# DanielLin94144/E2E-ASR-Pytorch

Measured on AMD Instinct MI355X. Metric: audio frames/sec (fwd+bwd) LibriSpeech-100 joint CTC-att, higher is better.
Workload: dtype bf16; 1 GPU; config/librispeech_asr.yaml (vgg 0, 4xBiLSTM-320, joint CTC-att 0.5), B=16 x T=1200 x D=160 per GPU, L=180, delta+SpecAugment on GPU, fwd+losses+bwd+grad-allreduce+clip+Adadelta, dropout on; global_batch=16, frames_per_utt=1200, parallelism=dp1

## Files before the change

### e2e-asr-pytorch_amd/csrc/ctc.hip

```cpp
#include "common.h"

namespace {

struct CtcP {
    const float* lp;
    const int64_t* tgt;
    const int64_t* in_len;
    const int64_t* tgt_len;
    float* nll;
    float* loss;
    float* grad;
    float* alpha;
    float* beta;
    int B, T, V, L, Smax;
    float gscale;
};

__device__ __forceinline__ float lse2(float a, float b) {
    const float m = fmaxf(a, b);
    if (m == -INFINITY) return -INFINITY;
    return m + __logf(1.f + __expf(-fabsf(a - b)));
}

__device__ __forceinline__ float lse3(float a, float b, float c) {
    const float m = fmaxf(fmaxf(a, b), c);
    if (m == -INFINITY) return -INFINITY;
    const float md = __builtin_amdgcn_fmed3f(a, b, c), mn = fminf(fminf(a, b), c);
    return m + __logf(1.f + __expf(md - m) + __expf(mn - m));
}

constexpr int CTC_FCH = 8;
constexpr size_t CTC_GRAD_LDS = 60 * 1024;

__global__ __launch_bounds__(1024) void ctc_sweep_kernel(CtcP p, int CF) {
    extern __shared__ __attribute__((aligned(16))) unsigned char smem[];
    const int b = blockIdx.x, back = blockIdx.y;
    const int tid = threadIdx.x, NTH = blockDim.x;
    const int V = p.V, T = p.T;
    int tl = (int)p.tgt_len[b];
    tl = max(0, min(tl, p.L));
    const int S = 2 * tl + 1;
    int Tin = (int)p.in_len[b];
    Tin = max(0, min(Tin, T));
    int* ext = reinterpret_cast<int*>(smem);
    float* buf0 = reinterpret_cast<float*>(ext + p.Smax + 2) + 2;
    float* buf1 = buf0 + p.Smax + 6;
    float* s_lp = buf1 + p.Smax + 4;
    const float* lp = p.lp + (long)b * T * V;
    float* lat = (back ? p.beta : p.alpha) + (long)b * T * p.Smax;

    for (int s = tid; s < p.Smax + 2; s += NTH) ext[s] = (s < S && (s & 1)) ? (int)p.tgt[(long)b * p.L + (s >> 1)] : 0;
    for (int s = tid - 2; s < p.Smax + 2; s += NTH) { buf0[s] = -INFINITY; buf1[s] = -INFINITY; }
    __syncthreads();
    if (Tin == 0) {
        if (!back && tid == 0) {
            const float n = (tl == 0) ? 0.f : INFINITY;
            p.nll[b] = n;
        }
        return;
    }
    const int nwb = (p.L + 1 + 63) >> 6;
    const bool label = (tid >> 6) >= nwb;
    const int s = label ? 2 * (tid - 64 * nwb) + 1 : 2 * tid;
    const bool sok = s < S;
    const int sr = sok ? s : 0;
    const int e = sok ? ext[s] : 0;
    bool skip = false;
    if (sok && !back) skip = (s >= 2) && e != 0 && e != ext[s - 2];
    if (sok && back) skip = (s + 2 < S) && ext[s + 2] != 0 && ext[s + 2] != e;
    float* prev = buf0;
    float* cur = buf1;
    for (int c0 = 0; c0 < Tin; c0 += CF) {
        const int nf = min(CF, Tin - c0);
        const int tlo = back ? Tin - c0 - nf : c0;
        __syncthreads();
        for (int i = tid; i < nf * V; i += NTH) s_lp[i] = lp[(long)tlo * V + i];
        __syncthreads();
        for (int i = 0; i < nf; ++i) {
            const int t = back ? Tin - 1 - (c0 + i) : c0 + i;
            const float lpe = s_lp[(t - tlo) * V + e];
            float a;
            if (c0 + i == 0) {
                if (!back) a = (s == 0 || s == 1) ? lpe : -INFINITY;
                else       a = (s == S - 1 || s == S - 2) ? lpe : -INFINITY;
            } else {
                const int d1 = back ? 1 : -1;
                if (label) a = lse3(prev[sr], prev[sr + d1], skip ? prev[sr + 2 * d1] : -INFINITY);
                else       a = lse2(prev[sr], prev[sr + d1]);
                a += lpe;
            }
            if (sok) { cur[s] = a; lat[(long)t * p.Smax + s] = a; }
            __syncthreads();
            float* tmp = prev; prev = cur; cur = tmp;
        }
    }
    if (!back && tid == 0) {
        float ll = prev[S - 1];
        if (S > 1) ll = lse2(ll, prev[S - 2]);
        p.nll[b] = -ll;
    }
}

template <int FCH>
__global__ __launch_bounds__(1024) void ctc_grad_kernel(CtcP p) {
    extern __shared__ __attribute__((aligned(16))) unsigned char smem[];
    const int b = blockIdx.y, t0 = blockIdx.x * FCH;
    const int tid = threadIdx.x, NTH = blockDim.x, lane = tid & 63, wave = tid >> 6, nwave = NTH >> 6;
    const int V = p.V, T = p.T;
    int tl = (int)p.tgt_len[b];
    tl = max(0, min(tl, p.L));
    const int S = 2 * tl + 1;
    int Tin = (int)p.in_len[b];
    Tin = max(0, min(Tin, T));
    float* acc = reinterpret_cast<float*>(smem);
    float* blk = acc + FCH * V;
    const float* lp = p.lp + (long)b * T * V;
    float* grad = p.grad + (long)b * T * V;
    for (int i = tid; i < FCH * V; i += NTH) acc[i] = 0.f;
    const int s = tid;
    const bool sok = s < S;
    const int e = (sok && (s & 1)) ? (int)p.tgt[(long)b * p.L + (s >> 1)] : 0;
    const float nll = p.nll[b];
    const float scale = p.gscale / (float)(max(tl, 1) * p.B);
    if (blockIdx.x == 0 && blockIdx.y == 0 && tid == 0) {
        float sum = 0.f;
        for (int bb = 0; bb < p.B; ++bb) {
            int l = (int)p.tgt_len[bb];
            l = max(1, min(l, p.L));
            sum += p.nll[bb] / (float)(l * p.B);
        }
        *p.loss = sum;
    }
    float occ[FCH];
#pragma unroll
    for (int f = 0; f < FCH; ++f) {
        const int t = t0 + f;
        occ[f] = 0.f;
        if (sok && t < Tin) {
            const long li = ((long)b * T + t) * p.Smax + s;
            occ[f] = expf(p.alpha[li] + p.beta[li] - lp[(long)t * V + e] + nll);
        }
    }
    __syncthreads();
#pragma unroll
    for (int f = 0; f < FCH; ++f) {
        if (sok && (s & 1) && t0 + f < Tin) atomicAdd(&acc[f * V + e], occ[f]);
        const float bsum = wave_sum((sok && !(s & 1)) ? occ[f] : 0.f);
        if (lane == 0) blk[f * nwave + wave] = bsum;
    }
    __syncthreads();
    for (int i = tid; i < FCH * V; i += NTH) {
        const int f = i / V, v = i - f * V, t = t0 + f;
        if (t >= T) continue;
        float g = 0.f;
        if (t < Tin) {
            float a = acc[i];
            if (v == 0) for (int w = 0; w < nwave; ++w) a += blk[f * nwave + w];
            if (!(nll < INFINITY)) a = NAN;
            g = scale * (expf(lp[(long)t * V + v]) - a);
        }
        grad[(long)t * V + v] = g;
    }
}

}

extern "C" size_t asr_ctc_loss_workspace_bytes(int B, int T, int L) {
    return 2 * (size_t)B * T * (2 * (size_t)L + 1) * sizeof(float);
}

extern "C" int asr_ctc_loss(const float* logp, const int64_t* targets, const int64_t* input_len, const int64_t* target_len,
                            float* nll, float* loss, float* grad, int B, int T, int V, int L, float gscale,
                            void* workspace, size_t workspace_bytes, asr_stream_t stream) {
    ASR_REQUIRE(logp && targets && input_len && target_len && nll && loss && grad && workspace, ASR_E_ARG, "asr_ctc_loss: null pointer");
    ASR_REQUIRE(B > 0 && T > 0 && V > 1 && L > 0, ASR_E_ARG, "asr_ctc_loss: bad dims");
    ASR_REQUIRE(workspace_bytes >= asr_ctc_loss_workspace_bytes(B, T, L), ASR_E_ARG, "asr_ctc_loss: workspace too small");
    const int Smax = 2 * L + 1;
    float* wsf = (float*)workspace;
    CtcP p{logp, targets, input_len, target_len, nll, loss, grad, wsf, wsf + (size_t)B * T * Smax, B, T, V, L, Smax, gscale};
    ASR_REQUIRE(Smax <= 1024, ASR_E_UNSUPPORTED, "asr_ctc_loss: 2L+1=%d states exceed one workgroup", Smax);
    const int nthr = 64 * ((L + 1 + 63) / 64 + (L + 63) / 64);
    const size_t fixed = (size_t)(Smax + 2) * 4 + 2 * (size_t)(Smax + 6) * 4 + 16;
    int CF = (int)((60 * 1024 - fixed) / ((size_t)V * 4));
    ASR_REQUIRE(CF >= 1, ASR_E_UNSUPPORTED, "asr_ctc_loss: V=%d classes exceed the LDS budget: at most V=%d with 2L+1=%d states "
                "(one frame of log-probs beside the lattice buffers in 60 KB)", V, (int)((60 * 1024 - fixed) / 4), Smax);
    if (CF > T) CF = T;
    const size_t lds_s = fixed + (size_t)CF * V * 4;
    const size_t lds_g1 = (size_t)(V + nthr / 64) * 4;
    ASR_REQUIRE(lds_g1 <= CTC_GRAD_LDS, ASR_E_UNSUPPORTED, "asr_ctc_loss: V=%d classes exceed the %zu bytes of LDS of the gradient kernel",
                V, CTC_GRAD_LDS);
    int fch = CTC_FCH;
    while ((size_t)fch * lds_g1 > CTC_GRAD_LDS) fch >>= 1;
    hipStream_t st = (hipStream_t)stream;
    hipLaunchKernelGGL(ctc_sweep_kernel, dim3(B, 2), dim3(nthr), lds_s, st, p, CF);
    const dim3 gg(cdiv(T, fch), B);
    switch (fch) {
        case 8: hipLaunchKernelGGL(ctc_grad_kernel<8>, gg, dim3(nthr), 8 * lds_g1, st, p); break;
        case 4: hipLaunchKernelGGL(ctc_grad_kernel<4>, gg, dim3(nthr), 4 * lds_g1, st, p); break;
        case 2: hipLaunchKernelGGL(ctc_grad_kernel<2>, gg, dim3(nthr), 2 * lds_g1, st, p); break;
        default: hipLaunchKernelGGL(ctc_grad_kernel<1>, gg, dim3(nthr), lds_g1, st, p); break;
    }
    ASR_LAUNCH_CHECK("asr_ctc_loss");
    return ASR_OK;
}
```

### e2e-asr-pytorch_amd/csrc/decoder.hip

```cpp
#include "common.h"
#include "gemm_plan.h"
#include "decoder_internal.h"
#include <stdlib.h>
#include <initializer_list>
#include <type_traits>

namespace {

template <typename F> void with_bool(bool v, F&& f) { if (v) f(std::true_type{}); else f(std::false_type{}); }
template <typename F> void with_knmax_h16(int Kn, bool h16, F&& f) {
    with_bool(h16, [&](auto h) {
        if (Kn <= 4) f(std::integral_constant<int, 4>{}, h);
        else if (Kn <= 10) f(std::integral_constant<int, 10>{}, h);
        else f(std::integral_constant<int, 16>{}, h);
    });
}

__host__ __device__ inline int conv_parts(int nout) { const int p = 512 / nout; return p < 1 ? 1 : (p > 8 ? 8 : p); }

__device__ __forceinline__ float tanh_fast(float x) { return 1.f - 2.f * __builtin_amdgcn_rcpf(1.f + __expf(2.f * x)); }

template <int U> struct Stage {
    float v[U];
    template <typename L> __device__ __forceinline__ void load(int n, int tid, int nthr, L ld) {
// ... 1046 lines not shown
    o.ntp_max = pi.tiles_max;
    o.slots = take((size_t)d.B * (o.nte > o.ntp_max ? o.nte : o.ntp_max) * o.slot);
    o.pwork_bytes = pi.work_bytes;
    o.pwork = take(o.pwork_bytes / sizeof(float) + 64);
    o.dxin = take((size_t)d.B * d.L * XW);
    o.dkeypre = take((size_t)d.B * d.Tp * d.A);
    o.datt_next = take((size_t)d.B * d.Tp);
    o.dcf = take((size_t)d.NL * d.B * d.Dd);
    o.wq_t = take((size_t)d.Q * d.A);
    o.wslots = take((size_t)d.B * o.nch * d.Kn * taps);
    for (int l = 0; l < d.NL; ++l) o.wcat[l] = take((size_t)((l == 0 ? XW : d.Dd) + d.Dd) * 4 * d.Dd);
    o.total = off;
    return o;
}

int check_dims(const asr_dec_dims_t& d, const char* who) {
    ASR_REQUIRE(d.B > 0 && d.Tp > 0 && d.E > 0 && d.A > 0 && d.Dd > 0 && d.V > 1 && d.L > 0, ASR_E_ARG, "%s: bad dims", who);
    ASR_REQUIRE(d.NL >= 1 && d.NL <= ASR_MAX_DEC_LAYERS, ASR_E_UNSUPPORTED, "%s: %d decoder layers (max %d)", who, d.NL, ASR_MAX_DEC_LAYERS);
    ASR_REQUIRE(d.Q == d.Dd * d.NL, ASR_E_ARG, "%s: Q must equal Dd*NL", who);
    ASR_REQUIRE(d.Kn >= 1 && d.Kn <= 16, ASR_E_UNSUPPORTED, "%s: loc_kernel_num %d not in [1,16]", who, d.Kn);
    ASR_REQUIRE(d.Ks >= 0 && d.Ks <= 512, ASR_E_UNSUPPORTED, "%s: loc_kernel_size %d too large", who, d.Ks);
    ASR_REQUIRE(d.temperature > 0.f, ASR_E_ARG, "%s: temperature must be > 0", who);
    ASR_REQUIRE(d.Tp <= 12000, ASR_E_UNSUPPORTED, "%s: T'=%d exceeds the LDS row budget", who, d.Tp);
    return ASR_OK;
}

struct EnergyPlan { int tpw; dim3 grid; size_t lds; };
EnergyPlan energy_plan(const asr_dec_dims_t& d) {
    const int cand_small[] = {2, 4, 5, 8}, cand_big[] = {2, 4, 5};
    const int* cand = (d.Kn <= 4) ? cand_small : cand_big;
    const int nc = (d.Kn <= 4) ? 4 : (d.Kn <= 10 ? 3 : 2);
    int tpw = cand[nc - 1];
    for (int i = 0; i < nc; ++i)
        if ((long)d.B * cdiv(d.Tp, 8 * cand[i]) <= 256) { tpw = cand[i]; break; }
    EnergyPlan pl;
    pl.tpw = tpw;
    const int TE = 8 * tpw;
    pl.grid = dim3(cdiv(d.Tp, TE), d.B);
    int n[5];
    energy_regions(TE, d.Kn, d.Ks, d.A, n);
    n[4] = conv_parts(d.Kn * (TE / 4)) * d.Kn * TE;
    pl.lds = lds_bytes(n, 5);
    return pl;
}
void launch_energy(const DecP& p, int t, const EnergyPlan& pl, hipStream_t st) {
    with_knmax_h16(p.d.Kn, p.s.key16 != nullptr, [&](auto kn, auto h) {
        constexpr int KNMAX = decltype(kn)::value;
        constexpr bool H16 = decltype(h)::value;
        switch (pl.tpw) {
            case 2: hipLaunchKernelGGL((att_energy_kernel<KNMAX, 2, H16>), pl.grid, dim3(512), pl.lds, st, p, t); break;
            case 4: hipLaunchKernelGGL((att_energy_kernel<KNMAX, 4, H16>), pl.grid, dim3(512), pl.lds, st, p, t); break;
            case 5: if constexpr (KNMAX <= 10) { hipLaunchKernelGGL((att_energy_kernel<KNMAX, 5, H16>), pl.grid, dim3(512), pl.lds, st, p, t); } break;
            default: if constexpr (KNMAX <= 4) { hipLaunchKernelGGL((att_energy_kernel<KNMAX, 8, H16>), pl.grid, dim3(512), pl.lds, st, p, t); } break;
        }
    });
}

void launch_step(const DecP& p, int t, bool bf, const EnergyPlan& epl, bool embed, hipStream_t st) {
    const asr_dec_dims_t& d = p.d;
    if (embed)
        hipLaunchKernelGGL(embed_kernel, dim3(cdiv((long)d.B * d.Dd, 256)), dim3(256), 0, st, p.w.emb, p.s.tokens, p.s.xin, d.B, d.L, d.Dd,
                           d.Dd + d.E, t, 1, d.V);
    with_bool(bf, [&](auto b) { hipLaunchKernelGGL(dec_query_kernel<decltype(b)::value>, dim3(cdiv(d.A, 16)), dim3(256), 0, st, p, t); });
    launch_energy(p, t, epl, st);
    if (p.s.enc16 && (d.E & 3) == 0) hipLaunchKernelGGL(att_softmax_ctx_kernel<true>, dim3(cdiv(d.E, 64), d.B), dim3(256), sizeof(float) * d.Tp, st, p, t);
    else hipLaunchKernelGGL(att_softmax_ctx_kernel<false>, dim3(cdiv(d.E, 64), d.B), dim3(256), sizeof(float) * d.Tp, st, p, t);
    for (int l = 0; l < d.NL; ++l)
        with_bool(bf, [&](auto b) { hipLaunchKernelGGL(dec_cell_fwd_kernel<decltype(b)::value>, dim3(cdiv(d.Dd, 4)), dim3(256), 0, st, p, t, l); });
}

GemmCall key_call(const asr_dec_dims_t& d, const asr_dec_weights_t& w, const float* enc, float* key, int prec) {
    GemmCall c{enc, w.Wk, key, w.bk, d.B * d.Tp, d.A, d.E, d.E, d.E, d.A};
    c.act = ASR_ACT_TANH; c.prec = prec;
    return c;
}

}

extern "C" size_t asr_att_decoder_fwd_work_bytes(const asr_dec_dims_t* dims) {
    return dims ? dec_fwd_plan_info(*dims).work_bytes : 0;
}
extern "C" int asr_att_decoder_fwd_plan(const asr_dec_dims_t* dims) { return dims ? dec_fwd_plan_info(*dims).kind : 0; }
extern "C" int asr_att_decoder_bwd_plan(const asr_dec_dims_t* dims) { return dims ? dec_bwd_plan_info(*dims).kind : 0; }
extern "C" int asr_att_decoder_energy_plan(const asr_dec_dims_t* dims, int* knmax, int* tpw) {
    ASR_REQUIRE(dims && knmax && tpw, ASR_E_ARG, "asr_att_decoder_energy_plan: null pointer");
    const int rc = check_dims(*dims, "asr_att_decoder_energy_plan");
    if (rc != ASR_OK) return rc;
    with_knmax_h16(dims->Kn, false, [&](auto kn, auto) { *knmax = decltype(kn)::value; });
    *tpw = energy_plan(*dims).tpw;
    return ASR_OK;
}

static __global__ void dec_fwd_begin_kernel(unsigned* status, int has_block) {
    status[threadIdx.x] = 0u;
    if (has_block && threadIdx.x == 0) status[DEC_FWD_LAUNCHED_WORD] = 0u;
}

extern "C" int asr_att_decoder_fwd(const asr_dec_dims_t* dims, const asr_dec_weights_t* weights,
                                   const float* enc, const int64_t* enc_len, const int64_t* teacher, int teacher_ld,
                                   const asr_dec_state_t* state, int prec, asr_stream_t stream) {
    ASR_REQUIRE(dims && weights && enc && enc_len && state, ASR_E_ARG, "asr_att_decoder_fwd: null pointer");
    const asr_dec_dims_t& d = *dims;
    int rc = check_dims(d, "asr_att_decoder_fwd");
    if (rc != ASR_OK) return rc;
    hipStream_t st = (hipStream_t)stream;
    DecP p{d, *weights, *state, enc, enc_len};
    const bool bf = (prec == ASR_BF16);
    if (state->work && state->work_bytes >= 256)
        hipLaunchKernelGGL(dec_fwd_begin_kernel, dim3(1), dim3(64), 0, st, (unsigned*)state->work, state->work_bytes >= DEC_STATUS_BYTES ? 1 : 0);

    rc = gemm_run(key_call(d, *weights, enc, state->key, prec), st);
    if (rc != ASR_OK) return rc;
    if (state->key16) hipLaunchKernelGGL(cast_bf16_kernel, dim3(1024), dim3(256), 0, st, state->key, (unsigned short*)state->key16, (long)d.B * d.Tp * d.A);
    if (state->enc16) hipLaunchKernelGGL(cast_bf16_kernel, dim3(1024), dim3(256), 0, st, enc, (unsigned short*)state->enc16, (long)d.B * d.Tp * d.E);

    if (teacher) {
        hipLaunchKernelGGL(shift_tokens_kernel, dim3(cdiv(d.B * d.L, 256)), dim3(256), 0, st, teacher, state->tokens, d.B, d.L, teacher_ld);
        hipLaunchKernelGGL(embed_kernel, dim3(cdiv((long)d.B * d.L * d.Dd, 256)), dim3(256), 0, st, weights->emb, state->tokens,
                           state->xin, d.B, d.L, d.Dd, d.Dd + d.E, 0, d.L, d.V);
    } else {
        hipMemsetAsync(state->tokens, 0, sizeof(int64_t) * d.B * d.L, st);
    }

    const EnergyPlan epl = energy_plan(d);
    ASR_REQUIRE(epl.lds <= 64 * 1024, ASR_E_UNSUPPORTED, "asr_att_decoder_fwd: energy tile needs %zu B of LDS", epl.lds);
    int t_begin = 0;
    if (teacher && bf && state->work) {
        rc = dec_fwd_persistent(d, *weights, *state, enc, enc_len, state->work, state->work_bytes, st);
        if (rc < 0) return rc;
        if (rc == ASR_OK) t_begin = d.L;
    }
    for (int t = t_begin; t < d.L; ++t) {
        launch_step(p, t, bf, epl, !teacher, st);
        if (!teacher) hipLaunchKernelGGL(dec_greedy_kernel, dim3(d.B), dim3(256), 0, st, p, t);
    }
    ASR_LAUNCH_CHECK("asr_att_decoder_fwd");
    if (teacher) {
        GemmCall logits{state->hs + (size_t)(d.NL - 1) * d.Dd, weights->Wc, state->logits, weights->bc, d.B * d.L, d.V, d.Dd,
                        (long)d.NL * d.Dd, d.Dd, d.V};
        logits.prec = prec;
        rc = gemm_run(logits, st);
        if (rc != ASR_OK) return rc;
    }
    return ASR_OK;
}

extern "C" int asr_att_decoder_keys(const asr_dec_dims_t* dims, const asr_dec_weights_t* weights, const float* enc,
                                    float* key, int prec, asr_stream_t stream) {
    ASR_REQUIRE(dims && weights && enc && key, ASR_E_ARG, "asr_att_decoder_keys: null pointer");
    return gemm_run(key_call(*dims, *weights, enc, key, prec), (hipStream_t)stream);
}

extern "C" int asr_att_decoder_step(const asr_dec_dims_t* dims, const asr_dec_weights_t* weights,
                                    const float* enc, const int64_t* enc_len, const asr_dec_state_t* state, int t,
                                    int prec, asr_stream_t stream) {
    ASR_REQUIRE(dims && weights && enc && enc_len && state, ASR_E_ARG, "asr_att_decoder_step: null pointer");
    const asr_dec_dims_t& d = *dims;
    int rc = check_dims(d, "asr_att_decoder_step");
    if (rc != ASR_OK) return rc;
    ASR_REQUIRE(t >= 0 && t < d.L, ASR_E_ARG, "asr_att_decoder_step: step %d outside [0,%d)", t, d.L);
    hipStream_t st = (hipStream_t)stream;
    DecP p{d, *weights, *state, enc, enc_len};
    const EnergyPlan epl = energy_plan(d);
    ASR_REQUIRE(epl.lds <= 64 * 1024, ASR_E_UNSUPPORTED, "asr_att_decoder_step: energy tile needs %zu B of LDS", epl.lds);
    launch_step(p, t, prec == ASR_BF16, epl, true, st);
    ASR_LAUNCH_CHECK("asr_att_decoder_step");
    if (d.V > DEC_LOGITS_ROW_MAX_V) {
        GemmCall logits{state->hs + ((size_t)t * d.NL + (d.NL - 1)) * d.Dd, weights->Wc, state->logits + (size_t)t * d.V, weights->bc,
                        d.B, d.V, d.Dd, (long)d.L * d.NL * d.Dd, d.Dd, (long)d.L * d.V};
        logits.prec = prec;
        return gemm_run(logits, st);
    }
    hipLaunchKernelGGL(dec_logits_kernel, dim3(d.B), dim3(256), 0, st, p, t);
    ASR_LAUNCH_CHECK("asr_att_decoder_step");
    return ASR_OK;
}

extern "C" size_t asr_att_decoder_bwd_status_offset(const asr_dec_dims_t* dims) {
    if (!dims) return 0;
    return bwd_layout(*dims).pwork;
}

extern "C" int asr_att_decoder_bwd_persistent_tiles(const asr_dec_dims_t* dims) {
    if (!dims) return 0;
    return bwd_layout(*dims).ntp;
}

extern "C" size_t asr_att_decoder_bwd_workspace_bytes(const asr_dec_dims_t* dims) {
// ... 301 lines not shown
```

### e2e-asr-pytorch_amd/csrc/decoder_cluster.h

```cpp
#pragma once
#include "common.h"
#include "handoff.h"
#include "decoder_internal.h"
#include <stdlib.h>
#include <algorithm>

namespace {


constexpr u64 PAIR_MASK = 7ull | (7ull << 32);
__device__ __forceinline__ u64 pair_want(unsigned seq, unsigned epoch) {
    epoch = 2u + epoch % 14u;
    const unsigned tag = ((epoch & 15u) << 2) | seq;
    return (u64)(tag & 7u) | ((u64)(tag >> 3) << 32);
}
__device__ __forceinline__ u64 pack2(float a, float b, u64 want) {
    return ((u64)(__float_as_uint(a) & ~7u) | ((u64)(__float_as_uint(b) & ~7u) << 32)) | want;
}
__device__ __forceinline__ float lo_f(u64 g) { return __uint_as_float((unsigned)g & ~7u); }
__device__ __forceinline__ float hi_f(u64 g) { return __uint_as_float((unsigned)(g >> 32) & ~7u); }
__device__ __forceinline__ unsigned f2h_bits(float x) { return (unsigned)__builtin_bit_cast(unsigned short, (_Float16)x); }
__device__ __forceinline__ u64 pack4h(float a, float b, float c, float d, u64 want) {
    const unsigned lo = (f2h_bits(a) & ~7u) | (f2h_bits(b) << 16), hi = (f2h_bits(c) & ~7u) | (f2h_bits(d) << 16);
    return ((u64)lo | ((u64)hi << 32)) | want;
}
__device__ __forceinline__ float h2f_lo(unsigned w) { return (float)__builtin_bit_cast(_Float16, (unsigned short)(w & 0xffffu)); }
__device__ __forceinline__ float h2f_hi(unsigned w) { return (float)__builtin_bit_cast(_Float16, (unsigned short)(w >> 16)); }
constexpr float NEG_BIG = -1e30f;
constexpr int NCW = 8, NPW = 4;
constexpr int FSW_NU = 3;
constexpr int FCVX_LD = 32;
#ifdef ASR_DIAG
#define DP_DECL unsigned long long dg_t = __builtin_amdgcn_s_memrealtime(), dg_acc[16] = {0, 0, 0, 0, 0, 0, 0, 0, 0, 0, 0, 0, 0, 0, 0, 0};
#define DP_MARK(k) { __builtin_amdgcn_sched_barrier(0); asm volatile("s_waitcnt lgkmcnt(0)" ::: "memory"); unsigned long long n_ = __builtin_amdgcn_s_memrealtime(); dg_acc[k] += n_ - dg_t; dg_t = n_; __builtin_amdgcn_sched_barrier(0); }
#define DP_DUMP { if (blockIdx.x == 0 && threadIdx.x == 0) { unsigned long long* o = (unsigned long long*)p.status + 128; for (int k = 0; k < 16; ++k) o[k] = dg_acc[k]; } }
#define DP_JIT(k)
#elif defined(ASR_JITTER)
__device__ __forceinline__ void dp_jitter(unsigned k, unsigned step, unsigned epoch) {
    unsigned h = (blockIdx.x * 0x9E3779B1u) ^ ((threadIdx.x >> 6) * 0x85EBCA6Bu) ^ (k * 0xC2B2AE35u) ^ (step * 0x27D4EB2Fu) ^ (epoch * 0x165667B1u);
    h ^= h >> 15; h *= 0x2C1B3C6Du; h ^= h >> 12; h *= 0x297A2D39u; h ^= h >> 15;
    h = __builtin_amdgcn_readfirstlane(h);
    if ((h & 3u) == 0u) {
        const unsigned n = (h >> 2) & 63u;
        for (unsigned i = 0; i < n; ++i) __builtin_amdgcn_s_sleep(4);
    }
}
#define DP_DECL
#define DP_MARK(k) dp_jitter(k, (unsigned)t, epoch_);
#define DP_JIT(k) dp_jitter(32 + k, (unsigned)t, epoch_);
#define DP_DUMP
#else
#define DP_DECL
#define DP_MARK(k)
#define DP_JIT(k)
#define DP_DUMP
#endif

__device__ __forceinline__ float wave_sum_dpp(float v) {
#define DPB_STEP(CTRL, RMASK) v += __builtin_bit_cast(float, __builtin_amdgcn_update_dpp(0, __builtin_bit_cast(int, v), CTRL, RMASK, 0xf, false));
    DPB_STEP(0xB1, 0xf)
    DPB_STEP(0x4E, 0xf)
    DPB_STEP(0x141, 0xf)
    DPB_STEP(0x140, 0xf)
    DPB_STEP(0x142, 0xa)
    DPB_STEP(0x143, 0xc)
#undef DPB_STEP
    return __builtin_bit_cast(float, __builtin_amdgcn_readlane(__builtin_bit_cast(int, v), 63));
}
__device__ __forceinline__ float sum8_dpp(float v) {
    v += __builtin_bit_cast(float, __builtin_amdgcn_update_dpp(0, __builtin_bit_cast(int, v), 0xB1, 0xf, 0xf, false));
    v += __builtin_bit_cast(float, __builtin_amdgcn_update_dpp(0, __builtin_bit_cast(int, v), 0x4E, 0xf, 0xf, false));
    v += __builtin_bit_cast(float, __builtin_amdgcn_update_dpp(0, __builtin_bit_cast(int, v), 0x141, 0xf, 0xf, false));
    return v;
}
__device__ __forceinline__ float sum16_dpp(float v) {
    v = sum8_dpp(v);
    v += __builtin_bit_cast(float, __builtin_amdgcn_update_dpp(0, __builtin_bit_cast(int, v), 0x140, 0xf, 0xf, false));
    return v;
}
__device__ __forceinline__ float wave_max_dpp(float v) {
#define DPB_STEP(CTRL, RMASK) v = fmaxf(v, __builtin_bit_cast(float, __builtin_amdgcn_update_dpp(__builtin_bit_cast(int, v), __builtin_bit_cast(int, v), CTRL, RMASK, 0xf, false)));
    DPB_STEP(0xB1, 0xf)
    DPB_STEP(0x4E, 0xf)
    DPB_STEP(0x141, 0xf)
    DPB_STEP(0x140, 0xf)
    DPB_STEP(0x142, 0xa)
    DPB_STEP(0x143, 0xc)
#undef DPB_STEP
    return __builtin_bit_cast(float, __builtin_amdgcn_readlane(__builtin_bit_cast(int, v), 63));
}

struct PD {
    asr_dec_dims_t d;
    asr_dec_weights_t w;
    asr_dec_state_t s;
    const float* enc;
    const int64_t* enc_len;
    const unsigned short* wcat16;
    const float* embproj;
    u64* xbuf;
    unsigned* status;
    int NT, TE, UPW, QPW, CPW;
    int HG2, QG2, SG2;
    int KC, KCP;
    int allow_local;
    unsigned epoch;
};

struct ConvGeo { int NKS, WKP, IMG_LD, need; };
__host__ __device__ inline ConvGeo conv_geo(int TEB, int Ks) {
    ConvGeo g;
    g.NKS = (2 * Ks + 1 + 31) >> 5;
    g.WKP = 32 * g.NKS + 8;
    g.need = ((TEB + 15) & ~15) + 32 * g.NKS + 8;
    g.IMG_LD = ((g.need - 32 + 127) / 128) * 128 + 32;
    return g;
}
__host__ __device__ inline int conv_img_shorts(const ConvGeo& g) { return 8 * g.IMG_LD + 32 * g.WKP; }

struct FCarve { int cvx_shorts, img, shorts, WT, ATP, NG, x2, q, wg, attp, wc, epart, e, w, g, cpart, stage, stage_floats, floats; };
__host__ __device__ inline FCarve fwd_carve(int TEB, int NT, int A, int E, int Kn, int Ks, int KCP, int UPW, int SG2) {
    FCarve c;
    c.cvx_shorts = TEB * FCVX_LD;
    c.img = (c.cvx_shorts + 7) & ~7;
    c.shorts = (c.img + conv_img_shorts(conv_geo(TEB, Ks)) + 7) & ~7;
    c.WT = (2 * Ks + 1 + 3) & ~3;
    c.ATP = (NT * TEB + 2 * Ks + 8 + 3) & ~3;
    const int nch = E >> 3;
    c.NG = (64 * NCW) / nch; if (c.NG > 8) c.NG = 8;
    int o = 0;
    c.x2 = o; o += 2 * KCP;
    c.q = o; o += (A + 3) & ~3;
    c.wg = o; o += (A + 3) & ~3;
    c.attp = o; o += c.ATP;
    c.wc = o;
    c.epart = o; o += NCW * TEB;
    c.e = o; o += TEB;
    c.w = o; o += TEB;
    c.g = o; o += (4 * UPW + 3) & ~3;
    c.cpart = o; o += c.NG * E;
    c.stage = o;
    c.stage_floats = NT * 2 * SG2; if (c.stage_floats < Kn * TEB) c.stage_floats = Kn * TEB;
    o += c.stage_floats;
    c.floats = o;
    return c;
}

__device__ inline void conv_build_wimg(const float* __restrict__ Wconv, int Kn, int taps, const ConvGeo& g, unsigned short* wimg, int tid, int nthr) {
    for (int i = tid; i < 16 * g.WKP; i += nthr) {
        const int n = i / g.WKP, x = i - n * g.WKP;
        const float v = (n < Kn && x < taps) ? Wconv[n * taps + x] : 0.f;
        const __bf16 hi = (__bf16)v, lo = (__bf16)(v - (float)hi);
        wimg[i] = __builtin_bit_cast(unsigned short, hi);
        wimg[16 * g.WKP + i] = __builtin_bit_cast(unsigned short, lo);
    }
}

__device__ inline void conv_build_ximg(const float* src, int navail, const ConvGeo& g, unsigned short* ximg, int tz, int nthr) {
    const int ngrp = g.IMG_LD >> 2;
    for (int it = tz; it < 4 * ngrp; it += nthr) {
        const int c = it / ngrp, gq = it - c * ngrp;
        unsigned short h[4], l[4];
#pragma unroll
        for (int e = 0; e < 4; ++e) {
            const int i = 4 * gq + c + e;
            const float v = (i < navail && i < g.need) ? src[i] : 0.f;
            const __bf16 hi = (__bf16)v, lo = (__bf16)(v - (float)hi);
            h[e] = __builtin_bit_cast(unsigned short, hi); l[e] = __builtin_bit_cast(unsigned short, lo);
        }
        *reinterpret_cast<uint2*>(ximg + (long)c * g.IMG_LD + 4 * gq) = make_uint2((unsigned)h[0] | ((unsigned)h[1] << 16), (unsigned)h[2] | ((unsigned)h[3] << 16));
        *reinterpret_cast<uint2*>(ximg + (long)(4 + c) * g.IMG_LD + 4 * gq) = make_uint2((unsigned)l[0] | ((unsigned)l[1] << 16), (unsigned)l[2] | ((unsigned)l[3] << 16));
    }
}

template <int NW, class Epi>
__device__ inline void conv_mfma(const unsigned short* ximg, const unsigned short* wimg, const ConvGeo& g, int MTB, int wave, int lane, Epi epi) {
    constexpr int CT = 3;
    const int m = lane & 15, q = lane >> 4, cc = m & 3;
    const unsigned short* xh = ximg + (long)cc * g.IMG_LD + (m - cc) + 8 * q;
    const unsigned short* xl = xh + 4 * g.IMG_LD;
    const unsigned short* wh = wimg + m * g.WKP + 8 * q;
    const unsigned short* wl = wh + 16 * g.WKP;
    for (int mt0 = wave; mt0 < MTB; mt0 += NW * CT) {
        f32x4 acc[CT];
#pragma unroll
        for (int c = 0; c < CT; ++c) acc[c] = f32x4{0.f, 0.f, 0.f, 0.f};
        for (int ks = 0; ks < g.NKS; ++ks) {
            const bf16x8 bh = *reinterpret_cast<const bf16x8*>(wh + 32 * ks), bl = *reinterpret_cast<const bf16x8*>(wl + 32 * ks);
#pragma unroll
            for (int c = 0; c < CT; ++c) {
                const int mt = mt0 + NW * c;
                if (mt < MTB) {
                    const unsigned short* ph = xh + 16 * mt + 32 * ks;
                    const unsigned short* pl = xl + 16 * mt + 32 * ks;
                    const uint2 h0 = *reinterpret_cast<const uint2*>(ph), h1 = *reinterpret_cast<const uint2*>(ph + 4);
                    const uint2 l0 = *reinterpret_cast<const uint2*>(pl), l1 = *reinterpret_cast<const uint2*>(pl + 4);
                    const bf16x8 ah = __builtin_bit_cast(bf16x8, make_uint4(h0.x, h0.y, h1.x, h1.y));
                    const bf16x8 al = __builtin_bit_cast(bf16x8, make_uint4(l0.x, l0.y, l1.x, l1.y));
                    acc[c] = mma16(bh, ah, acc[c]);
                    acc[c] = mma16(bl, ah, acc[c]);
                    acc[c] = mma16(bh, al, acc[c]);
                }
            }
        }
#pragma unroll
        for (int c = 0; c < CT; ++c) {
            const int mt = mt0 + NW * c;
            if (mt < MTB) epi(mt, m, q, acc[c]);
        }
    }
}

__device__ __forceinline__ void compute_barrier(unsigned* cnt, unsigned& gen) {
    gen += NCW;
    __builtin_amdgcn_fence(__ATOMIC_RELEASE, "workgroup");
    if ((threadIdx.x & 63) == 0) {
        __hip_atomic_fetch_add(cnt, 1u, __ATOMIC_RELAXED, __HIP_MEMORY_SCOPE_WORKGROUP);
        while (__hip_atomic_load(cnt, __ATOMIC_RELAXED, __HIP_MEMORY_SCOPE_WORKGROUP) < gen) __builtin_amdgcn_s_sleep(1);
    }
    __builtin_amdgcn_fence(__ATOMIC_ACQUIRE, "workgroup");
}

__global__ void build_wcat16_kernel(const float* __restrict__ wih, const float* __restrict__ whh, unsigned short* __restrict__ out,
                                    int rows, int Dd, int E, int KCP) {
    const long total = (long)rows * KCP;
    for (long i = blockIdx.x * (long)blockDim.x + threadIdx.x; i < total; i += (long)gridDim.x * blockDim.x) {
        const int r = (int)(i / KCP), k = (int)(i - (long)r * KCP);
        float v = 0.f;
        if (k < E) v = wih[(long)r * (Dd + E) + Dd + k];
        else if (k < E + Dd) v = whh[(long)r * Dd + (k - E)];
        out[i] = f2bf_bits(v);
    }
}

template <typename K>
bool grid_resident(K kernel, int grid, int block, size_t lds) {
    int per_cu = 0;
    if (hipOccupancyMaxActiveBlocksPerMultiprocessor(&per_cu, kernel, block, lds) != hipSuccess || per_cu < 1) return false;
    int dev = 0, cus = 0;
    if (hipGetDevice(&dev) != hipSuccess || hipDeviceGetAttribute(&cus, hipDeviceAttributeMultiprocessorCount, dev) != hipSuccess) return false;
    return grid <= cus;
}

template <int CH>
__device__ __forceinline__ void poll_copy(const u64* src, int n16, float* dst, int gt, int np, u64 want, unsigned* status) {
    for (int i0 = gt; i0 < n16; i0 += CH * np) {
        u64 lo[CH], hi[CH];
        int cnt = 0;
#pragma unroll
        for (int k = 0; k < CH; ++k) if (i0 + k * np < n16) cnt = k + 1;
        gather16<CH>(src + 2 * i0, 2 * np, cnt, PAIR_MASK, want, lo, hi, status);
#pragma unroll
        for (int k = 0; k < CH; ++k)
            if (k < cnt) *reinterpret_cast<float4*>(dst + 4 * (long)(i0 + k * np)) = make_float4(lo_f(lo[k]), hi_f(lo[k]), lo_f(hi[k]), hi_f(hi[k]));
    }
}

constexpr int EPOCH_WORD = 1008;
constexpr size_t STATUS_CLEAR_BYTES = 4032;
__global__ void bump_epoch_kernel(unsigned* status) { status[EPOCH_WORD] = status[EPOCH_WORD] + 1u; status[DEC_FWD_LAUNCHED_WORD] = 1u; }
__global__ void clear_work_kernel(uint4* work, long n16) {
    for (long i = blockIdx.x * (long)blockDim.x + threadIdx.x; i < n16; i += (long)gridDim.x * blockDim.x)
        if (i < (long)(STATUS_CLEAR_BYTES / 16) || i >= 256) work[i] = make_uint4(0u, 0u, 0u, 0u);
}
inline void clear_work(void* work, size_t xbuf_bytes, hipStream_t st) {
    const long n16 = (long)((4096 + xbuf_bytes) / 16);
    hipLaunchKernelGGL(clear_work_kernel, dim3((unsigned)std::min<long>((n16 + 255) / 256, 2048)), dim3(256), 0, st, (uint4*)work, n16);
}

}
```

### e2e-asr-pytorch_amd/csrc/decoder_internal.h

```cpp
#pragma once
#include "common.h"

inline size_t align_up256(size_t x) { return (x + 255) & ~(size_t)255; }

struct DecPlanInfo {
    int kind;
    int tiles, tiles_max;
    size_t work_bytes;
};
DecPlanInfo dec_fwd_plan_info(const asr_dec_dims_t& d);
DecPlanInfo dec_bwd_plan_info(const asr_dec_dims_t& d);
int dec_fwd_persistent(const asr_dec_dims_t& d, const asr_dec_weights_t& w, const asr_dec_state_t& s, const float* enc,
                       const int64_t* enc_len, void* work, size_t work_bytes, hipStream_t st);
constexpr int DEC_FWD_LAUNCHED_WORD = 1009;
constexpr size_t DEC_STATUS_BYTES = 4096;
int dec_bwd_persistent(const asr_dec_dims_t& d, const asr_dec_weights_t& w, const asr_dec_state_t& s, const int64_t* enc_len,
                       const float* dhs, float* dxin, float* dq, float* dkey, float* slots, int slot, const float* wcatT, const float* wqT,
                       void* work, size_t work_bytes, float** dgates_out, hipStream_t st);
float* dec_bwd_dgates(const asr_dec_dims_t& d, void* work);

int dec_fwd_streamed(const asr_dec_dims_t& d, const asr_dec_weights_t& w, const asr_dec_state_t& s, const float* enc,
                     const int64_t* enc_len, void* work, size_t work_bytes, hipStream_t st);
int dec_bwd_streamed(const asr_dec_dims_t& d, const asr_dec_weights_t& w, const asr_dec_state_t& s, const int64_t* enc_len,
                     const float* dhs, float* dxin, float* dq, float* dkey, float* slots, int slot, const float* wcatT, const float* wqT,
                     void* work, size_t work_bytes, float** dgates_out, hipStream_t st);
```

### e2e-asr-pytorch_amd/csrc/decoder_persist.hip

```cpp
#include "decoder_plan.h"
#include "gemm_plan.h"
#include "decoder_fwd_common.h"

static int g_persist_fwd = -1, g_persist_bwd = -1;
static int g_stream_fwd = -1, g_stream_bwd = -1;
extern "C" int asr_att_decoder_set_persistent(int flags) {
    const int old = (g_persist_fwd != 0 ? 1 : 0) | (g_persist_bwd != 0 ? 2 : 0) | (g_stream_fwd > 0 ? 4 : 0) | (g_stream_bwd > 0 ? 8 : 0);
    g_persist_fwd = flags & 1; g_persist_bwd = (flags >> 1) & 1; g_stream_fwd = (flags >> 2) & 1; g_stream_bwd = (flags >> 3) & 1;
    return old;
}
static void read_switches() {
    if (g_persist_fwd < 0) g_persist_fwd = env_switch("ASR_DEC_PERSIST", 1);
    if (g_persist_bwd < 0) g_persist_bwd = env_switch("ASR_DEC_PERSIST_BWD", 1);
    if (g_stream_fwd < 0) g_stream_fwd = env_switch("ASR_DEC_STREAM", 0);
    if (g_stream_bwd < 0) g_stream_bwd = env_switch("ASR_DEC_STREAM", 0);
}
static FwdPlan fwd_plan(const asr_dec_dims_t& d) { read_switches(); return chosen_plan(persist_plan(d), stream_plan_f(d), g_stream_fwd); }
static BwdPlan bwd_plan(const asr_dec_dims_t& d) { read_switches(); return chosen_plan(persist_plan_b(d), stream_plan_b(d), g_stream_bwd); }

DecPlanInfo dec_fwd_plan_info(const asr_dec_dims_t& d) {
    read_switches();
    const FwdPlan r = persist_plan(d), s = stream_plan_f(d);
    return {chosen_plan(r, s, g_stream_fwd).kind, 0, 0, std::max(r.total, s.total)};
}
DecPlanInfo dec_bwd_plan_info(const asr_dec_dims_t& d) {
    read_switches();
    const BwdPlan r = persist_plan_b(d), s = stream_plan_b(d), pl = chosen_plan(r, s, g_stream_bwd);
    return {pl.kind, pl.NT, std::max(r.NT, s.NT), std::max(r.total, s.total)};
}
float* dec_bwd_dgates(const asr_dec_dims_t& d, void* work) { return bwd_work(d, bwd_plan(d), work).dgates; }

namespace {

size_t dec_fwd_persist_lds(int TE, int NT, int A, int E, int Ks, int KCP, int UPW, int SG2) {
    const int EPL = 16 * cdiv(TE, 16);
    const ConvGeo cg = conv_geo(EPL, Ks);
    const size_t shorts = (size_t)((TE * A + 7) & ~7)
                        + ((TE * E + 7) & ~7)
                        + EPL * FCVX_LD
                        + 8 * cg.IMG_LD
                        + 32 * cg.WKP;
    const size_t floats = (size_t)2 * KCP
                        + ((A + 3) & ~3)
                        + ((A + 3) & ~3)
                        + ((NT * TE + 2 * Ks + 8 + 3) & ~3)
                        + NCW * EPL
                        + ((4 * UPW + 3) & ~3)
                        + (size_t)NT * 2 * SG2;
    return 2 * shorts + 4 * floats;
}

template <int KNMAX, int TPW>
__global__ __launch_bounds__(64 * (NCW + NPW)) void dec_fwd_persist(PD p) {
    constexpr int TE = 8 * TPW;
    constexpr int MT = (TE + 15) / 16;
    constexpr int EPL = 16 * MT;
    extern __shared__ __attribute__((aligned(16))) unsigned char smem[];
    __shared__ unsigned s_bar;
    __shared__ float s_scale[NCW][32];
    const asr_dec_dims_t& d = p.d;
    const int id = blockIdx.x, xcd = id & 7, slot = id >> 3;
    const int cb = slot / p.NT, j = slot - cb * p.NT;
    const int b = cb * 8 + xcd;
    if (b >= d.B) return;
    const unsigned epoch_ = __builtin_amdgcn_readfirstlane(p.status[EPOCH_WORD]);
    const int tid = threadIdx.x, lane = tid & 63, wave = __builtin_amdgcn_readfirstlane(tid >> 6);
    const int NT = p.NT, A = d.A, E = d.E, Dd = d.Dd, Tp = d.Tp, Kn = d.Kn, Ks = d.Ks, L = d.L;
    const int taps = 2 * Ks + 1;
    const int tau0 = j * TE;
    const int len = min((int)p.enc_len[b], Tp);
    const int tmax = max(len - 1, 0);
    unsigned short* s_key = reinterpret_cast<unsigned short*>(smem);
    unsigned short* s_enc = s_key + ((TE * A + 7) & ~7);
    unsigned short* s_cvx = s_enc + ((TE * E + 7) & ~7);
    const ConvGeo cg_ = conv_geo(EPL, Ks);
    unsigned short* s_ximg = s_cvx + EPL * FCVX_LD;
    unsigned short* s_wimg = s_ximg + 8 * cg_.IMG_LD;
    float* s_x2 = reinterpret_cast<float*>(s_wimg + 32 * cg_.WKP);
    float* s_q = s_x2 + 2 * p.KCP;
    float* s_wg = s_q + ((A + 3) & ~3);
    const int WT = (taps + 3) & ~3;
    const int ATP = (NT * TE + 2 * Ks + 8 + 3) & ~3;
    float* s_attp = s_wg + ((A + 3) & ~3);
    float* s_epart = s_attp + ATP;
    float* s_g = s_epart + NCW * EPL;
    float* s_stage = s_g + ((4 * p.UPW + 3) & ~3);
    if (tid == 0) s_bar = 0u;
    FwdCl cl_ = fwd_cl(p, b, j, s_x2, s_q, s_attp, s_g, s_stage, &s_scale[0][0], epoch_);
    clear_own_records(cl_, tid, blockDim.x);
    __syncthreads();
    cl_.local = xcd_consensus(reinterpret_cast<u64*>(p.status) + 64 + b, NT, p.allow_local, p.status);
    const FwdCl& cl = cl_;

    for (int i = tid; i < TE * A; i += blockDim.x) {
        const int f = i / A, a = i - f * A;
        s_key[((long)(f >> 2) * A + a) * 4 + (f & 3)] = f2bf_bits(p.s.key[((long)b * Tp + min(tau0 + f, tmax)) * A + a]);
    }
    for (int i = tid; i < TE * E; i += blockDim.x) {
        const int f = i / E, c = i - f * E;
        s_enc[i] = f2bf_bits(p.enc[((long)b * Tp + min(tau0 + f, tmax)) * E + c]);
    }
    for (int i = tid; i < EPL * FCVX_LD; i += blockDim.x) s_cvx[i] = 0;
    conv_build_wimg(p.w.Wconv, Kn, taps, cg_, s_wimg, tid, blockDim.x);
    for (int i = tid; i < A; i += blockDim.x) s_wg[i] = p.w.wg[i];
    for (int i = tid; i < 2 * p.KCP; i += blockDim.x) s_x2[i] = 0.f;
    {
        const float uni = 1.f / (float)max(len, 1);
        for (int i = tid; i < ATP; i += blockDim.x) {
            const int tau = i - Ks;
            s_attp[i] = (tau >= 0 && tau < len) ? uni : 0.f;
        }
    }
    __syncthreads();

    if (wave >= NCW) {
        const int gt = tid - 64 * NCW, np = 64 * NPW;
        for (int t = 0; t < L; ++t) {
            if (t > 0) poll_h(cl, t, gt, np);
            DP_JIT(0)
            __syncthreads();
            DP_JIT(1)
            poll_q(cl, t, gt, np);
            DP_JIT(2)
            __syncthreads();
            DP_JIT(3)
            poll_s(cl, t, gt, np);
            DP_JIT(4)
            __syncthreads();
            DP_JIT(5)
        }
        return;
    }

    unsigned gen = 0;
    const float bg = p.w.bg[0];
    float c_state = 0.f;
    const int RPW = (4 * p.UPW + NCW - 1) / NCW;
    const int nu_cnt = (((A + 15) >> 4) - wave + NCW - 1) / NCW;
    bf16x8 wpx[FSW_NU];
    float wgu[FSW_NU];
    sweep_operands<KNMAX>(cl, wave, lane, wpx, wgu);
    constexpr int QR = 2;
    QRows<QR> qrows;
    query_rows_load(cl, wave, lane, qrows);
// ... 92 lines not shown
            const float m = wave_max_dpp(ev);
            const float wv = (ev > 0.5f * NEG_BIG) ? __expf(ev - m) : 0.f;
            const float ssum = wave_sum_dpp(wv);
            const int c2 = tz;
            float x0 = 0.f, x1 = 0.f;
            if (2 * c2 < E) {
#pragma unroll
                for (int f = 0; f < TE; ++f) {
                    const float wf = __builtin_bit_cast(float, __builtin_amdgcn_readlane(__builtin_bit_cast(int, wv), f));
                    const unsigned pr = *reinterpret_cast<const unsigned*>(s_enc + f * E + 2 * c2);
                    x0 += wf * __uint_as_float(pr << 16);
                    x1 += wf * __uint_as_float(pr & 0xffff0000u);
                }
            }
            u64* rec = st.out + cl.offS + (long)j * p.SG2;
            const int ghead = (TE + 2) >> 1;
            const float y0 = __shfl_down(x0, 1), y1 = __shfl_down(x1, 1);
            if (2 * c2 < E && (c2 & 1) == 0) {
                publish_gran(cl.local, rec + ghead + (c2 >> 1), pack4h(x0, x1, y0, y1, st.want));
            }
            if (wave == NCW - 1) {
                const float e0 = __shfl(ev, min(2 * lane, 63)), e1 = __shfl(ev, min(2 * lane + 1, 63));
                if (lane < TE / 2) {
                    publish_gran(cl.local, rec + lane, pack2(e0, e1, st.want));
                } else if (lane == TE / 2) {
                    publish_gran(cl.local, rec + lane, pack2(m, ssum, st.want));
                } else if (lane == TE / 2 + 1 && ghead + E / 4 < p.SG2) {
                    publish_gran(cl.local, rec + p.SG2 - 1, pack2(0.f, 0.f, st.want));
                }
            }
        }
        DP_MARK(7)
        __syncthreads();
        DP_MARK(8)
        combine_records(cl, st, TE);
        DP_MARK(9)
        compute_barrier(&s_bar, gen);
        DP_MARK(10)
        cell_rows<10>(cl, st, RPW, add_r);
        DP_MARK(11)
        compute_barrier(&s_bar, gen);
        DP_MARK(12)
        cell_update<false>(cl, st, c_state);
        DP_MARK(13)
    }
    DP_DUMP
}

FwdPlan persist_plan(const asr_dec_dims_t& d) {
    if (d.NL != 1 || d.B > 64 || d.A > 16 * FSW_NU * NCW || d.Kn > 10 || (d.E & 7) != 0 || d.Dd > 20 * 32 || d.Tp < 1) return FwdPlan{};
    const int cpx = cdiv(d.B, 8);
    const int cand[] = {2, 4, 5, 8};
    FwdPlan pl{};
    for (int i = 0; i < 4 && !pl.tpw; ++i) {
        const int nt = cdiv(d.Tp, 8 * cand[i]);
        if (nt <= 30 && cpx * nt <= 32) pl.tpw = cand[i];
    }
    if (!pl.tpw) return FwdPlan{};
    pl.kind = 1; pl.TE = 8 * pl.tpw; pl.NT = cdiv(d.Tp, pl.TE);
    fwd_sizes(d, pl);
    if (pl.UPW > 64 || cdiv(4 * pl.UPW, NCW) > 60) return FwdPlan{};
    pl.lds = dec_fwd_persist_lds(pl.TE, pl.NT, d.A, d.E, d.Ks, pl.KCP, pl.UPW, pl.SG2);
    if (getenv("ASR_DEC_PLAN_DEBUG")) fprintf(stderr, "[asr] resident fwd plan B=%d T'=%d: NT=%d TE=%d UPW=%d LDS=%zu\n", d.B, d.Tp, pl.NT, pl.TE, pl.UPW, pl.lds);
    return pl.lds > 156 * 1024 ? FwdPlan{} : pl;
}

}

int dec_fwd_persistent(const asr_dec_dims_t& d, const asr_dec_weights_t& w, const asr_dec_state_t& s, const float* enc,
                       const int64_t* enc_len, void* work, size_t work_bytes, hipStream_t st) {
    read_switches();
    if (!g_persist_fwd) return 1;
    const FwdPlan pl = fwd_plan(d);
    if (pl.kind == 2) return dec_fwd_streamed(d, w, s, enc, enc_len, work, work_bytes, st);
    if (!pl.kind || !work || work_bytes < pl.total || ((uintptr_t)work & 255) != 0 || !s.conv) return 1;
    const FwdWork wk = fwd_work(d, pl, work);
    clear_work(work, wk.xbuf_bytes, st);
    hipLaunchKernelGGL(build_wcat16_kernel, dim3(512), dim3(256), 0, st, w.Wih[0], w.Whh[0], wk.wcat16, 4 * d.Dd, d.Dd, d.E, pl.KCP);
    const int XW = d.Dd + d.E;
    GemmCall embproj{s.xin, w.Wih[0], wk.embproj, nullptr, d.B * d.L, 4 * d.Dd, d.Dd, XW, XW, 4 * d.Dd};
    embproj.prec = ASR_BF16;
    int rc = gemm_run(embproj, st);
    if (rc != ASR_OK) return rc;
    const PD p{d, w, s, enc, enc_len, wk.wcat16, wk.embproj, wk.xbuf, wk.status, pl.NT, pl.TE, pl.UPW, pl.QPW, pl.CPW, pl.HG2, pl.QG2, pl.SG2, pl.KC,
               pl.KCP, xcd_local_allowed()};
    const ClusterLaunch go{"asr_att_decoder_fwd(persistent)", 160 * 1024 - 2048, cluster_grid(d, pl.NT), dim3(64 * (NCW + NPW)), pl.lds, st};
    if (d.Kn <= 4) {
        if (pl.tpw == 2) return go.run<dec_fwd_persist<4, 2>>(p);
        if (pl.tpw == 4) return go.run<dec_fwd_persist<4, 4>>(p);
        if (pl.tpw == 5) return go.run<dec_fwd_persist<4, 5>>(p);
        return go.run<dec_fwd_persist<4, 8>>(p);
    }
    if (pl.tpw == 2) return go.run<dec_fwd_persist<10, 2>>(p);
    if (pl.tpw == 4) return go.run<dec_fwd_persist<10, 4>>(p);
    if (pl.tpw == 5) return go.run<dec_fwd_persist<10, 5>>(p);
    return 1;
}

namespace {

template <int KNMAX, int TEC>
__global__ __launch_bounds__(512) void dec_bwd_persist(PB p) {
    extern __shared__ __attribute__((aligned(16))) unsigned char smem[];
    __shared__ unsigned s_bar;
    __shared__ float s_red[8];
    constexpr int KP = (KNMAX + 3) & ~3;
    const int TE = TEC ? TEC : p.TE;
    const int MT = (TE + 15) / 16;
    const asr_dec_dims_t& d = p.d;
    const int id = blockIdx.x, xcd = id & 7, slot_id = id >> 3;
    const int cb = slot_id / p.NT, j = slot_id - cb * p.NT;
    const int b = cb * 8 + xcd;
    if (b >= d.B) return;
    const unsigned epoch_ = __builtin_amdgcn_readfirstlane(p.status[EPOCH_WORD]);
    const int tid = threadIdx.x, lane = tid & 63, wave = __builtin_amdgcn_readfirstlane(tid >> 6);
    const int NT = p.NT, A = d.A, E = d.E, Dd = d.Dd, Tp = d.Tp, Kn = d.Kn, Ks = d.Ks, L = d.L;
    const int ncw = (A + 63) >> 6, nct = 64 * ncw, nw = ncw + NPB;
    const int taps = 2 * Ks + 1, XW = Dd + E, R4 = p.R4;
    const int tau0 = j * TE;
    const int len = min((int)p.enc_len[b], Tp);
    const int tmax = max(len - 1, 0);
    const BCarve cv_ = bwd_carve(TE, KP, A, E, Kn, Ks, NT, p.UPW, p.CG2, p.QG2, p.NG2);
    const int AP = cv_.AP, DW = cv_.DW, PADL = cv_.PADL, WT = cv_.WT, AQ = cv_.AQ;
    const int TW = NT * TE;
    const int CG2f = 2 * p.CG2, NG2f = 2 * p.NG2, QG2f = 2 * p.QG2;
    unsigned short* s_sh = reinterpret_cast<unsigned short*>(smem);
    unsigned short* s_key = s_sh + cv_.key;
    unsigned short* s_dl = s_sh + cv_.dl;
    unsigned short* s_wp16 = s_sh + cv_.wp16;
    unsigned short* s_dg16 = s_sh + cv_.dg16;
    unsigned short* s_wq16 = s_sh + cv_.wq16;
    unsigned short* s_cvx = s_sh + cv_.cvx;
    unsigned short* s_cvT = s_sh + cv_.cvT;
    float* s_f = reinterpret_cast<float*>(s_sh + cv_.shorts);
    float* s_wc = s_f + cv_.wc;
    float* s_crec = s_f + cv_.crec;
    float* s_qst = s_f + cv_.qst;
    float* s_nrec = s_f + cv_.nrec;
    float* s_dcp = s_f + cv_.dcp;
    float* s_de = s_f + cv_.de;
    float* s_out = s_f + cv_.out;
    float* s_hq = s_f + cv_.hq;
    float* s_pt = s_f + cv_.pt;
    float* s_dcx = s_f + cv_.dcx;
    float* s_dq = s_f + cv_.dq;
    const long region = (long)NT * (p.CG2 + p.QG2 + p.VG2 + p.NG2);
    auto xb = [&](int parity) { return p.xbuf + ((long)parity * d.B + b) * region; };
    const long offC = 0, offQ = offC + (long)NT * p.CG2, offV = offQ + (long)NT * p.QG2, offN = offV + (long)NT * p.VG2;
    if (tid == 0) s_bar = 0u;
    for (int parity = 0; parity < 2; ++parity) {
        u64* base = xb(parity);
        for (int i = tid; i < p.CG2; i += blockDim.x) st_gran_local(base + offC + (long)j * p.CG2 + i, 0ull);
        for (int i = tid; i < p.QG2; i += blockDim.x) st_gran_local(base + offQ + (long)j * p.QG2 + i, 0ull);
        for (int i = tid; i < p.VG2; i += blockDim.x) st_gran_local(base + offV + (long)j * p.VG2 + i, 0ull);
        for (int i = tid; i < p.NG2; i += blockDim.x) st_gran_local(base + offN + (long)j * p.NG2 + i, 0ull);
    }
    asm volatile("s_waitcnt vmcnt(0)" ::: "memory");
    __syncthreads();
    const bool local = xcd_consensus(reinterpret_cast<u64*>(p.status) + 64 + b, NT, p.allow_local, p.status);

    for (int i = tid; i < TE * A; i += blockDim.x) {
        const int f = i / A, a = i - f * A;
        s_key[((long)(f >> 2) * A + a) * 4 + (f & 3)] = f2bf_bits(p.s.key[((long)b * Tp + min(tau0 + f, tmax)) * A + a]);
    }
    for (int i = tid; i < 16 * AP; i += blockDim.x) { const int k = i / AP, a = i - k * AP; s_wp16[i] = (k < Kn && a < A) ? f2bf_bits(p.w.Wproj[a * Kn + k]) : (unsigned short)0; }
    for (int i = tid; i < Kn * WT; i += blockDim.x) { const int k = i / WT, jj = i - k * WT; s_wc[i] = (jj < taps) ? p.w.Wconv[k * taps + jj] : 0.f; }
    for (int i = tid; i < 64 * KCHB * 4; i += blockDim.x) s_dg16[i] = 0;
    for (int i = tid; i < NT * NG2f + 8; i += blockDim.x) s_nrec[i] = 0.f;
    for (int i = tid; i < NT * CG2f; i += blockDim.x) s_crec[i] = 0.f;
    for (int i = tid; i < Kn * DW; i += blockDim.x) s_dcp[i] = 0.f;
    for (int i = tid; i < TE * AP; i += blockDim.x) s_dl[i] = 0;
    for (int i = tid; i < 16 * SW_MT * CVX_LD; i += blockDim.x) s_cvx[i] = 0;
    for (int i = tid; i < 16 * CVT_LD; i += blockDim.x) s_cvT[i] = 0;
    for (int i = tid; i < 16 * SW_MT; i += blockDim.x) s_de[i] = 0.f;
    const int u_base = j * p.UPW, c_base = j * p.CPW;
    for (int i = tid; i < p.UPW * AQ; i += blockDim.x) {
        const int ul = i / AQ, aa = i - ul * AQ;
        s_wq16[i] = (aa < A && u_base + ul < Dd) ? f2bf_bits(p.wqT[(long)(u_base + ul) * A + aa]) : (unsigned short)0;
    }
// ... 322 lines not shown
```

### e2e-asr-pytorch_amd/src/asr.py

```python
import math

import torch
import torch.nn as nn

from src import functions as F_hip
from src import hipabi as H
from src.module import RNNLayer, Downsampler, LocationAwareAttention, LSTMParams
from src.util import init_weights_, init_gate_

ALIGN = 64


class _RunCtx(object):

    def __init__(self, model):
        self.anchor = model._anchor
        self.prec = model.prec
        self._model = model

    def next_seed(self):
        self._model._drop_counter += 1
        return (self._model.seed * 1000003 + self._model._drop_counter) & 0xFFFFFFFFFFFF


# ... 139 lines not shown
        sections.append(('rest', [[p] for p in self.parameters() if id(p) not in seen]))
        return sections

    def _flatten(self):
        params = list(self.parameters())
        if not params:
            return
        dev = params[0].device
        sections = self._param_groups_for_flat()
        offs, off, ranges = {}, 0, []
        for kind, groups in sections:
            start = (off + ALIGN - 1) // ALIGN * ALIGN
            for g in groups:
                off = (off + ALIGN - 1) // ALIGN * ALIGN
                for p in g:
                    offs[id(p)] = off
                    off += p.numel()
            off = (off + ALIGN - 1) // ALIGN * ALIGN
            ranges.append((kind, start, off))
        total = off
        flat = torch.zeros(total, dtype=torch.float32, device=dev)
        grad = torch.zeros(total, dtype=torch.float32, device=dev)
        for p in params:
            o, n = offs[id(p)], p.numel()
            flat[o:o + n].copy_(p.data.reshape(-1))
            p.data = flat[o:o + n].view(p.shape)
            p.grad = grad[o:o + n].view(p.shape)
            p._asr_flat = (flat, grad, offs)
        self.flat_param, self.flat_grad, self._offsets, self._ranges = flat, grad, offs, ranges
        self._anchor = torch.zeros(1, dtype=torch.float32, device=dev, requires_grad=True)

        def view_of(ps, shape, is_grad):
            o = offs[id(ps[0])]
            n = sum(p.numel() for p in ps)
            return (grad if is_grad else flat)[o:o + n].view(shape)
        for m in self.modules():
            if hasattr(m, 'bind_flat'):
                m.bind_flat(view_of)

    def attach_data_parallel(self, group=None, reducer_cls=None):
        from src.dist import FlatDataParallel
        if reducer_cls is not None:
            FlatDataParallel = reducer_cls
        rnn = [(s, e) for k, s, e in self._ranges if k == 'rnn']
        front = [(s, e) for k, s, e in self._ranges if k == 'front' and e > s]
        rest = [(s, e) for k, s, e in self._ranges if k == 'rest' and e > s]
        buckets = rest + rnn[::-1] + front
        dp = FlatDataParallel(self.flat_param, self.flat_grad, buckets, group)
        layers = [m for m in self.encoder.layers if isinstance(m, RNNLayer)]
        for i, m in enumerate(layers[::-1]):
            m.dp, m.bucket = dp, len(rest) + i
        for m in self.encoder.layers:
            if not isinstance(m, RNNLayer) and hasattr(m, 'bucket') and front:
                m.dp, m.bucket = dp, len(buckets) - 1
        self._dp, self._n_rest = dp, len(rest)
        return dp

    def _apply(self, fn, *args, **kwargs):
        super()._apply(fn, *args, **kwargs)
        self._flatten()
        return self

    def zero_grad(self, set_to_none=False):
        self.flat_grad.zero_()

    def set_state(self, prev_state, prev_attn):
        self.decoder.hidden_state = prev_state
        self.attention.att_layer.set_mem(prev_attn)

    def create_msg(self):
        msg = ['Model spec.| Encoder\'s downsampling rate of time axis is {}.'.format(self.encoder.sample_rate)]
        if self.encoder.vgg == 1:
            msg.append('           | VGG Extractor w/ time downsampling rate = 4 in encoder enabled.')
        if self.encoder.vgg == 5:
            msg.append('           | VGG Extractor w/ Layer normalization and downsampling rate = 4.')
        if self.enable_ctc:
            msg.append('           | CTC training on encoder enabled ( lambda = {}).'.format(self.ctc_weight))
        if self.enable_att:
            msg.append('           | {} attention decoder enabled ( lambda = {}).'.format(self.attention.mode, 1 - self.ctc_weight))
        msg.append('           | HIP path (gfx950), contraction precision = {}.'.format('bf16' if self.prec == H.BF16 else 'fp32'))
        return msg

    def forward(self, audio_feature, feature_len, decode_step, tf_rate=0.0, teacher=None,
                emb_decoder=None, get_dec_state=False, get_logit=False, ctc_async=False):
        if not audio_feature.is_cuda:
            raise RuntimeError('ASR (HIP path) needs CUDA tensors; there is no CPU fallback')
        fuse_dec = (emb_decoder if emb_decoder is not None and getattr(emb_decoder, 'enable', False) and emb_decoder.apply_fuse
                    and teacher is None and self.enable_att else None)
        ctx = _RunCtx(self)
        feature_len = feature_len.to(audio_feature.device)
        ctc_output, att_output, att_seq, dec_state = None, None, None, None
        encode_feature, encode_len = self.encoder(audio_feature.float(), feature_len, ctx)
        encode_feature = F_hip.to_f32_fn(encode_feature)
        dp = getattr(self, '_dp', None)
        overlaps = H.step_overlaps(dp)
        side_ctc = (self.enable_ctc and self.enable_att and self.training and torch.is_grad_enabled() and overlaps
                    and H.ctc_side_enabled() and dp is None)
        if self.enable_ctc:
            if side_ctc:
                with H.side_branch(True, encode_feature, encode_len):
                    ctc_output = F_hip.CTCHeadFn.apply(ctx.anchor, encode_feature, self.ctc_layer[0], self.prec, get_logit, overlaps)
                ctc_output._asr_side = bool(ctc_async)
            else:
                ctc_output = F_hip.CTCHeadFn.apply(ctx.anchor, encode_feature, self.ctc_layer[0], self.prec, get_logit, overlaps)
        if self.enable_att:
            L = int(decode_step)
            if not (self.decoder.fast and self.attention.fast and self.emb_drop == 0.0):
                from src.variants import variant_decoder
                att_output, att_seq, hs = variant_decoder(self, ctx.anchor, encode_feature, encode_len, L, teacher,
                                                          float(tf_rate) if teacher is not None else 1.0, ctx, emb_decoder=fuse_dec)
                if get_dec_state:
                    dec_state = hs
                if side_ctc and not ctc_async:
                    H.join_branch(ctc_output)
                return ctc_output, encode_len, att_output, att_seq, dec_state
            if fuse_dec is not None:
                d, st, att_output = F_hip.att_decoder_forward_fused(self, encode_feature.contiguous(),
                                                                    encode_len.to(encode_feature.device, torch.int64).contiguous(), L,
                                                                    self.prec, fuse_dec)
                att_seq, hs = st['att'].view(d.B, 1, d.L, d.Tp), st['hs']
                self._last_tokens = st['tokens']
            else:
                att_output, att_seq, hs = F_hip.AttDecoderFn.apply(ctx.anchor, encode_feature, encode_len, teacher, L, self, self.prec,
                                                                   float(tf_rate) if teacher is not None else 1.0)
            if get_dec_state:
                dec_state = hs[:, :, -1, :]
        if side_ctc and not ctc_async:
            H.join_branch(ctc_output)
        return ctc_output, encode_len, att_output, att_seq, dec_state

    def fix_ctc_layer(self):
        for param in self.ctc_layer.parameters():
            param.requires_grad = False
```

### e2e-asr-pytorch_amd/src/functions.py

```python
import contextlib
import ctypes
import weakref

import torch

from src import hipabi as H


def _empty(shape, like):
    return torch.empty(shape, dtype=torch.float32, device=like.device)


def out_frames(layer, T):
    r = layer.sample_rate
    if r == 1:
        return T, 1
    return ((T + r - 1) // r, 1) if layer.sample_style == 'drop' else (T // r, r)


def _empty16(shape, like):
    return torch.empty(shape, dtype=torch.bfloat16, device=like.device)


def to_bf16(x):
# ... 373 lines not shown
    @staticmethod
    def forward(ctx, anchor, enc, lin, prec, get_logit, defer):
        enc = enc.contiguous()
        B, T, E = enc.shape
        V = lin.weight.shape[0]
        act = _empty((B, T, V), enc)
        H.linear_fwd(enc.view(B * T, E), lin.weight, lin.bias, act.view(B * T, V), act=H.ACT_RELU, prec=prec)
        ctx.lin, ctx.prec, ctx.get_logit, ctx.defer = lin, prec, get_logit, defer
        if get_logit:
            ctx.save_for_backward(enc, act)
            return act
        logp = _empty((B, T, V), enc)
        H.call('asr_log_softmax', H.ptr(act), H.ptr(logp), B * T, V, H.stream_ptr())
        ctx.save_for_backward(enc, act, logp)
        return logp

    @staticmethod
    def backward(ctx, g):
        lin, prec = ctx.lin, ctx.prec
        g = g.contiguous()
        if ctx.get_logit:
            enc, act = ctx.saved_tensors
            B, T, E = enc.shape
            V = act.shape[-1]
            dpre = _empty((B * T, V), enc)
            H.call('asr_act_bwd', H.ptr(g), H.ptr(act), H.ptr(dpre), B * T * V, H.ACT_RELU, H.stream_ptr())
        else:
            enc, act, logp = ctx.saved_tensors
            B, T, E = enc.shape
            V = act.shape[-1]
            dpre = _empty((B * T, V), enc)
            H.call('asr_logsoftmax_relu_bwd', H.ptr(g), H.ptr(logp), H.ptr(act), H.ptr(dpre), B * T, V, H.stream_ptr())
        denc = _empty((B, T, E), enc)
        if ctx.defer:
            H.linear_bwd_input(lin.weight, dpre, denc.view(B * T, E), prec=prec)
            x2d = enc.view(B * T, E)
            H.defer_side(lambda: H.linear_bwd(x2d, lin.weight, dpre, lin.weight.grad, lin.bias.grad, None, prec=prec), x2d, dpre)
        else:
            H.linear_bwd(enc.view(B * T, E), lin.weight, dpre, lin.weight.grad, lin.bias.grad, denc.view(B * T, E), prec=prec)
        return None, denc, None, None, None, None


def scale_by_device_scalar(x, alpha):
    x = x.contiguous()
    out = torch.empty_like(x)
    a = alpha.reshape(1).to(torch.float32).contiguous()
    H.call('asr_scale_dev', H.ptr(x), H.ptr(out), x.numel(), H.ptr(a), H.stream_ptr())
    return out


_LOSS_W = {}


def loss_weight(value, device):
    key = (float(value), str(device))
    if key not in _LOSS_W:
        _LOSS_W[key] = torch.full((1,), float(value), dtype=torch.float32, device=device)
    return _LOSS_W[key]


class LossMixFn(torch.autograd.Function):

    @staticmethod
    def forward(ctx, a, wa, b, wb):
        out = torch.empty((), dtype=torch.float32, device=a.device)
        H.call('asr_loss_mix', H.ptr(a), H.ptr(wa), H.ptr(b), H.ptr(wb) if b is not None else None, H.ptr(out), H.stream_ptr())
        ctx.has_b = b is not None
        ctx.save_for_backward(wa, *( [wb] if b is not None else []))
        return out

    @staticmethod
    def backward(ctx, g):
        sv = ctx.saved_tensors
        g = g.reshape(1).to(torch.float32).contiguous()
        ga = torch.empty((), dtype=torch.float32, device=g.device)
        H.call('asr_loss_mix', H.ptr(g), H.ptr(sv[0]), None, None, H.ptr(ga), H.stream_ptr())
        gb = None
        if ctx.has_b:
            gb = torch.empty((), dtype=torch.float32, device=g.device)
            H.call('asr_loss_mix', H.ptr(g), H.ptr(sv[1]), None, None, H.ptr(gb), H.stream_ptr())
        return ga, None, gb, None


class CTCLossFn(torch.autograd.Function):
    @staticmethod
    def forward(ctx, logp_btv, targets, input_len, target_len):
        logp = logp_btv.contiguous()
        B, T, V = logp.shape
        targets = targets.contiguous()
        L = targets.shape[1]
        if 2 * L + 1 > 1024:
            L = max(1, int(target_len.max()))
            targets = targets[:, :L].contiguous()
        dev = logp.device
        nll = torch.empty(B, dtype=torch.float32, device=dev)
        loss = torch.empty((), dtype=torch.float32, device=dev)
        grad = _empty((B, T, V), logp)
        nbytes = H.lib().asr_ctc_loss_workspace_bytes(B, T, L)
        ws = torch.empty(nbytes, dtype=torch.uint8, device=dev)
        targets = targets.to(dev, torch.int64)
        il = input_len.to(dev, torch.int64).contiguous()
        tl = target_len.to(dev, torch.int64).contiguous()
        H.call('asr_ctc_loss', H.ptr(logp), H.ptr(targets), H.ptr(il), H.ptr(tl), H.ptr(nll), H.ptr(loss), H.ptr(grad),
               B, T, V, L, 1.0, H.ptr(ws), nbytes, H.stream_ptr())
        ctx.save_for_backward(grad)
        ctx.nll = nll
        return loss

    @staticmethod
    def backward(ctx, gout):
        (grad,) = ctx.saved_tensors
        return scale_by_device_scalar(grad, gout), None, None, None


class SeqLossFn(torch.autograd.Function):
    @staticmethod
    def forward(ctx, logits_rv, target_r, mode, classes, smoothing):
        logits = logits_rv.contiguous()
        R, V = logits.shape
        tgt = target_r.to(logits_rv.device, torch.int64).contiguous()
        dev = logits.device
        dl = _empty((R, V), logits)
        loss = torch.empty((), dtype=torch.float32, device=dev)
        acc = torch.empty(4, dtype=torch.float32, device=dev)
        H.call('asr_xent', H.ptr(logits), H.ptr(tgt), R, H.ptr(dl), H.ptr(loss), H.ptr(acc), 1, R, V, mode, classes,
               smoothing, 1.0, H.stream_ptr())
        ctx.save_for_backward(dl)
        return loss

    @staticmethod
    def backward(ctx, gout):
        (dl,) = ctx.saved_tensors
        return scale_by_device_scalar(dl, gout), None, None, None, None


def _dec_dims(model, B, Tp, L):
    att, dec = model.attention, model.decoder
    d = H.DecDims()
    d.B, d.Tp, d.E = B, Tp, model.encoder.out_dim
    d.A, d.Q = att.dim, dec.dim * dec.layer
    d.Dd, d.NL, d.V = dec.dim, dec.layer, model.vocab_size
    d.Kn, d.Ks = att.att_layer.kernel_num, att.att_layer.kernel_size
    d.L = L
    d.temperature = float(att.att_layer.temperature)
    return d


def _dec_tensors(model, grads):
    att, dec, al = model.attention, model.decoder, model.attention.att_layer
    g = (lambda p: p.grad) if grads else (lambda p: p)
    nl = dec.layer
    return {
        'Wq': g(att.proj_q.weight), 'bq': g(att.proj_q.bias), 'Wk': g(att.proj_k.weight), 'bk': g(att.proj_k.bias),
        'Wconv': g(al.loc_conv.weight), 'Wproj': g(al.loc_proj.weight), 'wg': g(al.gen_energy.weight), 'bg': g(al.gen_energy.bias),
        'emb': g(model.pre_embed.weight),
        'Wih': [g(getattr(dec.layers, 'weight_ih_l%d' % l)) for l in range(nl)],
        'Whh': [g(getattr(dec.layers, 'weight_hh_l%d' % l)) for l in range(nl)],
        'bih': [g(getattr(dec.layers, 'bias_ih_l%d' % l)) for l in range(nl)],
        'bhh': [g(getattr(dec.layers, 'bias_hh_l%d' % l)) for l in range(nl)],
        'Wc': g(dec.char_trans.weight), 'bc': g(dec.char_trans.bias),
    }


def _dec_state(d, dev, save_conv=True, half_copies=False):
    f = lambda *s: torch.empty(s, dtype=torch.float32, device=dev)
    h = lambda *s: torch.empty(s, dtype=torch.bfloat16, device=dev)
    return {
        'conv': f(d.B, d.L, d.Kn, d.Tp) if save_conv else None,
        'key16': h(d.B, d.Tp, d.A) if half_copies else None,
        'enc16': h(d.B, d.Tp, d.E) if half_copies else None,
        'key': f(d.B, d.Tp, d.A), 'att': f(d.B, d.L, d.Tp), 'q': f(d.B, d.L, d.A), 'xin': f(d.B, d.L, d.Dd + d.E),
        'gates': f(d.B, d.L, d.NL, 4 * d.Dd), 'cs': f(d.B, d.L, d.NL, d.Dd), 'hs': f(d.B, d.L, d.NL, d.Dd),
        'logits': f(d.B, d.L, d.V), 'energy': f(d.B, d.Tp),
        'tokens': torch.empty((d.B, d.L), dtype=torch.int64, device=dev),
    }


class DecoderStepper(object):

    def __init__(self, model, enc, enc_len, L, prec, save_conv=False):
        self.enc, self.enc_len, self.prec = enc, enc_len, prec
        self.d = _dec_dims(model, enc.shape[0], enc.shape[1], L)
        self.sd = _dec_state(self.d, enc.device, save_conv=save_conv, half_copies=False)
        self.sd['tokens'].zero_()
        self.w = H.dec_weights_struct(_dec_tensors(model, False), self.d.NL)
        self.s = H.dec_state_struct(self.sd)
        H.call('asr_att_decoder_keys', ctypes.byref(self.d), ctypes.byref(self.w), H.ptr(enc), H.ptr(self.sd['key']), prec, H.stream_ptr())

    def step(self, t, live_rows=None):
        self.d.B = self.enc.shape[0] if live_rows is None else live_rows
        H.call('asr_att_decoder_step', ctypes.byref(self.d), ctypes.byref(self.w), H.ptr(self.enc), H.ptr(self.enc_len),
               ctypes.byref(self.s), t, self.prec, H.stream_ptr())


def att_decoder_forward_sampled(model, enc, enc_len, L, teacher, prec, tf_rate, decisions=None):
    dec = DecoderStepper(model, enc, enc_len, L, prec, save_conv=True)
    d, st = dec.d, dec.sd
    teacher = teacher.contiguous()
    model._ss_counter = getattr(model, '_ss_counter', 0)
    st['tf_decisions'] = []
    for t in range(L):
        dec.step(t)
        if t + 1 < L:
            use_teacher = bool(decisions[t]) if decisions is not None else (tf_rate == 1 or torch.rand(1).item() <= tf_rate)
            st['tf_decisions'].append(use_teacher)
            if use_teacher:
                st['tokens'][:, t + 1] = teacher[:, t]
            else:
                model._ss_counter += 1
                seed = (model.seed * 7919 + model._ss_counter) & 0xFFFFFFFFFFFF
                H.call('asr_sample_tokens', H.ptr(st['logits'][:, t]), st['logits'].stride(0), H.ptr(st['tokens'][:, t + 1]),
                       st['tokens'].stride(0), d.B, d.V, seed, H.stream_ptr())
    return d, st


@torch.no_grad()
def att_decoder_forward_fused(model, enc, enc_len, L, prec, emb_decoder):
    dec = DecoderStepper(model, enc, enc_len, L, prec)
    d, st = dec.d, dec.sd
    fused = torch.empty((d.B, L, d.V), dtype=torch.float32, device=enc.device)
    scratch = torch.empty(d.B, dtype=torch.int64, device=enc.device)
    for t in range(L):
        dec.step(t)
        nxt, ld = (st['tokens'][:, t + 1], st['tokens'].stride(0)) if t + 1 < L else (scratch, 1)
        row = emb_decoder.fuse_rows(st['hs'][:, t, -1, :], st['logits'][:, t], argmax=nxt, argmax_ld=ld)
        fused[:, t].copy_(row)
    return d, st, fused


_DEC_WS = {}


def _dec_workspace(model, kind, key, nbytes, device):
    dd = _dec_dims(model, *key)
    k = (kind, tuple(getattr(dd, f) for f, _ in dd._fields_), str(device))
    ws = _DEC_WS.pop(k, None)
    if ws is not None and ws.numel() < nbytes:
        H.handoff_release(ws)
        ws = None
    if ws is None:
        while len(_DEC_WS) >= 64:
            H.handoff_release(_DEC_WS.pop(next(iter(_DEC_WS))))
        ws = H.handoff_acquire(nbytes, device)
    _DEC_WS[k] = ws
    return ws


def att_decoder_forward(model, enc, enc_len, L, teacher, prec):
    B, Tp, _ = enc.shape
    d = _dec_dims(model, B, Tp, L)
    st = _dec_state(d, enc.device, half_copies=(prec == H.BF16 and d.E % 4 == 0))
    if prec == H.BF16 and teacher is not None:
        nwork = int(H.lib().asr_att_decoder_fwd_work_bytes(ctypes.byref(d)))
        if nwork:
            st['work'] = _dec_workspace(model, 'fwd', (d.B, d.Tp, d.L), nwork, enc.device)
            H.abort_guard(st['work'])
    w = H.dec_weights_struct(_dec_tensors(model, False), d.NL)
    s = H.dec_state_struct(st)
    t_ptr, t_ld = (None, 0)
    if teacher is not None:
        teacher = teacher.contiguous()
        assert teacher.shape[1] >= L - 1
        t_ptr, t_ld = H.ptr(teacher), teacher.shape[1]
    H.call('asr_att_decoder_fwd', ctypes.byref(d), ctypes.byref(w), H.ptr(enc), H.ptr(enc_len), t_ptr, t_ld,
           ctypes.byref(s), prec, H.stream_ptr())
    H.watch_abort(st.get('work'))
    return d, st


class AttDecoderFn(torch.autograd.Function):
    @staticmethod
    def forward(ctx, anchor, enc, enc_len, teacher, L, model, prec, tf_rate=1.0):
        enc = enc.contiguous()
        enc_len = enc_len.to(enc.device, torch.int64).contiguous()
        if teacher is not None and tf_rate != 1:
            d, st = att_decoder_forward_sampled(model, enc, enc_len, L, teacher, prec, tf_rate, getattr(model, '_tf_decisions', None))
            model._last_tokens = st['tokens']
        else:
            d, st = att_decoder_forward(model, enc, enc_len, L, teacher, prec)
        ctx.model, ctx.prec, ctx.d, ctx.st = model, prec, d, st
        ctx.save_for_backward(enc, enc_len)
        att_seq = st['att'].view(d.B, 1, d.L, d.Tp)
        ctx.mark_non_differentiable(att_seq)
        ctx.set_materialize_grads(False)
        return st['logits'], att_seq, st['hs']

    @staticmethod
    def backward(ctx, dlogits, _datt, dhs):
        model, prec, d, st = ctx.model, ctx.prec, ctx.d, ctx.st
        enc, enc_len = ctx.saved_tensors
        dlogits = torch.zeros_like(st['logits']) if dlogits is None else dlogits.contiguous()
        dhs_top = dhs[:, :, -1, :].contiguous() if dhs is not None else None
        denc = torch.zeros_like(enc)
        w = H.dec_weights_struct(_dec_tensors(model, False), d.NL)
        g = H.dec_weights_struct(_dec_tensors(model, True), d.NL)
        s = H.dec_state_struct(st)
        nbytes = H.lib().asr_att_decoder_bwd_workspace_bytes(ctypes.byref(d))
        ws = _dec_workspace(model, 'bwd', (d.B, d.Tp, d.L), nbytes, enc.device)
        model._last_dec_bwd_ws = ws
        persistent = int(H.lib().asr_att_decoder_bwd_persistent_tiles(ctypes.byref(d))) > 0
        status_off = int(H.lib().asr_att_decoder_bwd_status_offset(ctypes.byref(d))) if persistent else 0
        if persistent:
            H.abort_guard(ws, status_off)
        overlap = H.step_overlaps(getattr(model, '_dp', None))
        looped = ctypes.c_int(0)
        if dhs_top is None:
            H.call('asr_att_decoder_bwd_ex', ctypes.byref(d), ctypes.byref(w), ctypes.byref(g), H.ptr(enc), H.ptr(enc_len),
                   ctypes.byref(s), H.ptr(dlogits), H.ptr(denc), H.ptr(ws), nbytes, prec, 1 if overlap else 0, ctypes.byref(looped),
                   H.stream_ptr())
        else:
            H.call('asr_att_decoder_bwd_hs', ctypes.byref(d), ctypes.byref(w), ctypes.byref(g), H.ptr(enc), H.ptr(enc_len),
                   ctypes.byref(s), H.ptr(dlogits), H.ptr(dhs_top), H.ptr(denc), H.ptr(ws), nbytes, prec, 1 if overlap else 0,
                   ctypes.byref(looped), H.stream_ptr())
        if persistent:
            H.watch_abort(ws, status_off)
        if overlap:
            keep = [t for t in st.values() if torch.is_tensor(t)]

            def param_grads():
                H.call('asr_att_decoder_bwd_params', ctypes.byref(d), ctypes.byref(w), ctypes.byref(g), H.ptr(enc), H.ptr(enc_len),
                       ctypes.byref(s), H.ptr(dlogits), H.ptr(ws), nbytes, looped.value, prec, H.stream_ptr())
            H.defer_side(param_grads, enc, enc_len, dlogits, ws, *keep)
        ctx.st = None
        return None, denc, None, None, None, None, None, None


class EmbeddingFn(torch.autograd.Function):
    @staticmethod
    def forward(ctx, anchor, tokens, emb):
        tok = tokens.reshape(-1).contiguous()
        V, D = emb.weight.shape
        out = torch.empty((tok.numel(), D), dtype=torch.float32, device=tok.device)
        H.call('asr_gather_rows', H.ptr(emb.weight), H.ptr(tok), H.ptr(out), tok.numel(), D, D, D, V, H.stream_ptr())
        ctx.emb = emb
        ctx.save_for_backward(tok)
        return out.view(*tokens.shape, D)

    @staticmethod
    def backward(ctx, dout):
        (tok,) = ctx.saved_tensors
        emb = ctx.emb
        V, D = emb.weight.shape
        dout = dout.contiguous().view(-1, D)
        H.call('asr_embedding_bwd', H.ptr(dout), D, H.ptr(tok), H.ptr(emb.weight.grad), tok.numel(), D, V, H.stream_ptr())
        return None, None, None


class DropoutFn(torch.autograd.Function):

    @staticmethod
    def forward(ctx, x, p, seed):
        x = x.contiguous()
        B, T, D = x.shape
        z = torch.empty_like(x)
        H.call('asr_dropout_downsample_fwd', H.ptr(x), H.ptr(z), B, T, D, T, 1, 0, float(p), int(seed), H.stream_ptr())
        ctx.meta = (B, T, D, float(p), int(seed))
        return z

    @staticmethod
    def backward(ctx, dz):
        B, T, D, p, seed = ctx.meta
        dz = dz.contiguous()
        dx = torch.empty_like(dz)
        H.call('asr_dropout_downsample_bwd', H.ptr(dz), H.ptr(dx), B, T, D, T, 1, 0, p, seed, H.stream_ptr())
        return dx, None, None


class LinearFn(torch.autograd.Function):

    @staticmethod
    def forward(ctx, anchor, x, weight, bias, prec):
        x = x.contiguous()
        K = x.shape[-1]
        x2 = x.view(-1, K)
        N = weight.shape[0]
        out = torch.empty((x2.shape[0], N), dtype=torch.float32, device=x.device)
        H.linear_fwd(x2, weight, bias, out, prec=prec)
        ctx.weight, ctx.bias, ctx.prec = weight, bias, prec
        ctx.need_dx = x.requires_grad
        ctx.save_for_backward(x2)
        return out.view(*x.shape[:-1], N)

    @staticmethod
    def backward(ctx, dout):
        (x2,) = ctx.saved_tensors
        weight, bias, prec = ctx.weight, ctx.bias, ctx.prec
        N = weight.shape[0]
        dy = dout.contiguous().view(-1, N)
        dx = torch.empty_like(x2) if ctx.need_dx else None
        H.linear_bwd(x2, weight, dy, weight.grad, bias.grad if bias is not None else None, dx, prec=prec)
        return None, (dx.view(*dout.shape[:-1], x2.shape[1]) if dx is not None else None), None, None, None
```

### e2e-asr-pytorch_amd/src/hipabi.py

```python
import atexit
import contextlib
import ctypes
import os

import torch

_HERE = os.path.dirname(os.path.abspath(__file__))
LIB_PATH = os.environ.get('ASR_HIP_LIB') or os.path.join(os.path.dirname(_HERE), 'lib', 'libasr_hip.so')

F32, BF16 = 0, 1
ACT_NONE, ACT_TANH, ACT_RELU = 0, 1, 2
MAX_DEC_LAYERS = 4

_vp, _i, _l, _f, _u64, _sz = ctypes.c_void_p, ctypes.c_int, ctypes.c_long, ctypes.c_float, ctypes.c_uint64, ctypes.c_size_t


class DecDims(ctypes.Structure):
    _fields_ = [(n, _i) for n in ('B', 'Tp', 'E', 'A', 'Q', 'Dd', 'NL', 'V', 'Kn', 'Ks', 'L')] + [('temperature', _f)]


_DEC_W_FIELDS = ['Wq', 'bq', 'Wk', 'bk', 'Wconv', 'Wproj', 'wg', 'bg', 'emb']


class DecWeights(ctypes.Structure):
    _fields_ = [(n, _vp) for n in _DEC_W_FIELDS] + \
               [(n, _vp * MAX_DEC_LAYERS) for n in ('Wih', 'Whh', 'bih', 'bhh')] + [('Wc', _vp), ('bc', _vp)]


class DecState(ctypes.Structure):
    _fields_ = ([(n, _vp) for n in ('key', 'att', 'q', 'xin', 'gates', 'cs', 'hs', 'logits', 'energy', 'conv', 'key16', 'enc16', 'work')]
                + [('work_bytes', ctypes.c_size_t), ('tokens', _vp)])


class BeamStep(ctypes.Structure):
    _fields_ = ([(n, _vp) for n in ('att_logp', 'lm_logp', 'psi', 'candidates', 'alive_in', 'sum_in', 'ctcp_in', 'len_in', 'seq_in', 'score_in',
                                    'alive_out', 'sum_out', 'ctcp_out', 'len_out', 'seq_out', 'score_out', 'last_token', 'parent', 'ctc_index',
                                    'tokens')]
                + [('tokens_ld', _l)]
                + [(n, _vp) for n in ('min_len', 'max_len', 'done', 'fin_n', 'fin_len', 'fin_avg', 'fin_seq', 'fin_score')]
                + [(n, _i) for n in ('U', 'beam', 'V', 'C', 'Lmax', 't')]
                + [(n, _f) for n in ('ctc_weight', 'lm_weight', 'eos_threshold')])


ATT_DOT, ATT_LOC = 0, 1
BEAM_ATTEND_MAX_ROWS, BEAM_ATTEND_MAX_T = 16, 8192
CTC_BEAM_MAX = 16
BEAM_NARROW_MAX_V, BEAM_WIDE_MAX_V = 2048, 65536


class BeamAttend(ctypes.Structure):
    _fields_ = ([(n, _vp) for n in ('key', 'value', 'q', 'loc', 'wg', 'bg', 'enc_len', 'attn')] + [('attn_ld', _l), ('ctx', _vp)]
                + [(n, _l) for n in ('ctx_ld', 'ld_k', 'ld_v', 'ld_l')]
                + [(n, _i) for n in ('U', 'rows_per_utt', 'NH', 'NHv', 'Tp', 'A', 'Dv', 'mode', 'kv_bf16')] + [('temperature', _f)])


_P = ctypes.POINTER

SIGNATURES = {
    'asr_gemm': [_vp, _vp, _vp, _vp, _i, _i, _i, _l, _l, _l, _i, _i, _i, _i, _i, _i, _l, _l, _l, _i, _i, _i, _vp],
    'asr_lstm_fwd': [_vp, _vp, _vp, _vp, _vp, _i, _i, _i, _i, _i, _vp, _sz, _vp],
    'asr_lstm_bwd': [_vp, _vp, _vp, _vp, _i, _i, _i, _i, _i, _vp, _sz, _vp],
    'asr_dropout_downsample_fwd': [_vp, _vp, _i, _i, _i, _i, _i, _i, _f, _u64, _vp],
    'asr_dropout_downsample_bwd': [_vp, _vp, _i, _i, _i, _i, _i, _i, _f, _u64, _vp],
    'asr_dropout_mask': [_vp, _l, _f, _u64, _vp],
    'asr_act_bwd': [_vp, _vp, _vp, _l, _i, _vp],
    'asr_colsum': [_vp, _l, _i, _i, _vp, _vp],
    'asr_colsum2': [_vp, _l, _i, _i, _vp, _vp, _vp],
    'asr_log_softmax': [_vp, _vp, _l, _i, _vp],
    'asr_logsoftmax_relu_bwd': [_vp, _vp, _vp, _vp, _l, _i, _vp],
    'asr_layernorm_fwd': [_vp, _vp, _vp, _vp, _vp, _l, _i, _f, _i, _vp],
    'asr_layernorm_bwd': [_vp, _vp, _vp, _vp, _vp, _vp, _vp, _vp, _l, _i, _i, _vp],
    'asr_ctc_loss': [_vp, _vp, _vp, _vp, _vp, _vp, _vp, _i, _i, _i, _i, _f, _vp, _sz, _vp],
    'asr_xent': [_vp, _vp, _l, _vp, _vp, _vp, _i, _i, _i, _i, _i, _f, _f, _vp],
    'asr_att_decoder_fwd': [_P(DecDims), _P(DecWeights), _vp, _vp, _vp, _i, _P(DecState), _i, _vp],
    'asr_att_decoder_bwd': [_P(DecDims), _P(DecWeights), _P(DecWeights), _vp, _vp, _P(DecState), _vp, _vp, _vp, _sz, _i, _vp],
    'asr_att_decoder_bwd_ex': [_P(DecDims), _P(DecWeights), _P(DecWeights), _vp, _vp, _P(DecState), _vp, _vp, _vp, _sz, _i, _i,
                               ctypes.POINTER(_i), _vp],
    'asr_att_decoder_bwd_hs': [_P(DecDims), _P(DecWeights), _P(DecWeights), _vp, _vp, _P(DecState), _vp, _vp, _vp, _vp, _sz, _i, _i,
                               ctypes.POINTER(_i), _vp],
    'asr_emb_cos_loss': [_vp, _vp, _vp, _l, _vp, _vp, _vp, _vp, _i, _i, _i, _i, _vp],
    'asr_emb_fuse_fwd': [_vp, _l, _vp, _vp, _i, _vp, _i, _i, _vp, _vp, _vp, _l, _i, _i, _vp],
    'asr_emb_fuse_bwd': [_vp, _vp, _l, _vp, _vp, _i, _vp, _i, _i, _vp, _vp, _vp, _vp, _vp, _vp, _i, _i, _vp],
    'asr_row_normalize_fwd': [_vp, _vp, _l, _i, _vp],
    'asr_row_normalize_bwd': [_vp, _vp, _vp, _l, _i, _vp],
    'asr_att_decoder_bwd_params': [_P(DecDims), _P(DecWeights), _P(DecWeights), _vp, _vp, _P(DecState), _vp, _vp, _sz, _i, _i, _vp],
    'asr_fbank': [_vp, _vp, _vp, _vp, _vp, _vp, _i, _i, _i, _i, _i, _i, _i, _f, _f, _f, _vp, _sz, _vp],
    'asr_delta_stack': [_vp, _vp, _vp, _vp, _i, _i, _i, _i, _i, _vp],
    'asr_specaug': [_vp, _vp, _vp, _vp, _i, _i, _i, _i, _i, _u64, _vp],
    'asr_specaug_ws': [_vp, _vp, _vp, _vp, _i, _i, _i, _i, _i, _u64, _vp, _sz, _vp],
    'asr_cmvn': [_vp, _vp, _vp, _i, _i, _i, _f, _vp, _sz, _vp],
    'asr_specaug_policy': [_vp, _vp, _vp, _vp, _vp, _i, _i, _i, _i, _i, _i, _i, _i, _i, _i, _i, _u64, _vp, _sz, _vp],
    'asr_wave_draws': [_vp, _vp, _vp, _vp, _i, _i, _i, _u64, _vp],
    'asr_wave_noise': [_vp, _vp, _vp, _i, _i, _u64, _vp],
    'asr_wave_stft': [_vp, _vp, _vp, _i, _vp, _vp, _i, _i, _i, _vp],
    'asr_wave_pvoc': [_vp, _vp, _vp, _i, _vp, _i, _i, _i, _vp],
    'asr_wave_istft': [_vp, _vp, _vp, _i, _vp, _vp, _l, _i, _i, _i, _i, _vp],
    'asr_wave_resample': [_vp, _l, _vp, _vp, _i, _vp, _i, _i, _i, _vp],
    'asr_wave_augment': [_vp, _vp, _vp, _vp, _vp, _i, _i, _i, _u64, _vp, _sz, _vp],
    'asr_conv3x3': [_vp, _vp, _vp, _vp, _i, _i, _i, _i, _i, _i, _i, _i, _i, _vp],
    'asr_conv_weight_permute': [_vp, _vp, _i, _i, _i, _vp],
    'asr_vgg16_im2col': [_vp, _vp, _i, _i, _i, _i, _i, _vp],
    'asr_conv_weight_pack16': [_vp, _vp, _i, _i, _i, _i, _vp],
    'asr_conv_weight_fold': [_vp, _vp, _i, _i, _i, _vp],
    'asr_conv3x3_16': [_vp, _vp, _vp, _vp, _i, _i, _i, _i, _i, _i, _i, _i, _i, _vp],
    'asr_conv3x3_16_wgrad': [_vp, _vp, _vp, _i, _i, _i, _i, _i, _i, _i, _vp],
    'asr_maxpool2x2_16_fwd': [_vp, _vp, _vp, _i, _i, _i, _i, _i, _i, _vp],
    'asr_maxpool2x2_16_bwd': [_vp, _vp, _vp, _i, _i, _i, _i, _i, _i, _vp],
    'asr_ln_freq16_fwd': [_vp, _vp, _vp, _vp, _vp, _i, _i, _i, _i, _f, _i, _vp],
    'asr_ln_freq16_bwd': [_vp, _vp, _vp, _vp, _vp, _vp, _vp, _vp, _vp, _i, _i, _i, _i, _i, _vp],
    'asr_vgg16_output': [_vp, _vp, _i, _i, _i, _i, _vp],
    'asr_vgg16_output_bwd': [_vp, _vp, _i, _i, _i, _i, _vp],
    'asr_maxpool2x2_fwd': [_vp, _vp, _vp, _i, _i, _i, _i, _i, _i, _vp],
    'asr_maxpool2x2_bwd': [_vp, _vp, _vp, _i, _i, _i, _i, _i, _i, _vp],
    'asr_ln_freq_fwd': [_vp, _vp, _vp, _vp, _vp, _l, _i, _i, _f, _i, _vp],
# ... 16 lines not shown
    'asr_lstm_cell_fwd': [_vp, _vp, _vp, _i, _i, _vp, _vp, _vp, _vp],
    'asr_lstm_cell_bwd': [_vp, _vp, _vp, _vp, _vp, _i, _i, _vp, _vp, _vp],
    'asr_gru_cell_fwd': [_vp, _vp, _vp, _i, _i, _vp, _vp, _vp],
    'asr_gru_cell_bwd': [_vp, _vp, _vp, _i, _i, _vp, _vp, _vp, _vp],
    'asr_gru_fwd': [_vp, _vp, _vp, _i, _i, _i, _i, _vp, _vp, _vp],
    'asr_gru_bwd': [_vp, _vp, _vp, _vp, _i, _i, _i, _i, _vp, _vp, _vp],
    'asr_gru_rec_fwd': [_vp, _vp, _vp, _vp, _i, _i, _i, _i, _vp, _vp, _vp],
    'asr_gru_rec_bwd': [_vp, _vp, _vp, _vp, _vp, _i, _i, _i, _i, _vp, _vp, _vp, _vp, _sz, _vp],
    'asr_sumsq': [_vp, _l, _vp, _vp],
    'asr_scale': [_vp, _l, _f, _vp],
    'asr_scale_dev': [_vp, _vp, _l, _vp, _vp],
    'asr_loss_mix': [_vp, _vp, _vp, _vp, _vp, _vp],
    'asr_adadelta_step': [_vp, _vp, _vp, _vp, _l, _f, _f, _f, _f, _f, _vp, _f, _vp, _vp],
    'asr_adam_step': [_vp, _vp, _vp, _vp, _vp, _l, _f, _f, _f, _f, _f, _i, _f, _vp, _f, _vp, _vp, _vp],
    'asr_embedding_bwd': [_vp, _l, _vp, _vp, _i, _i, _i, _vp],
    'asr_status_collect': [ctypes.POINTER(_vp), _i, _vp, _vp],
    'asr_beam_candidates': [_vp, _vp, _i, _i, _i, _vp],
    'asr_sample_tokens': [_vp, _l, _vp, _l, _i, _i, _u64, _vp],
    'asr_beam_step': [ctypes.POINTER(BeamStep), _vp],
    'asr_beam_candidates_wide': [_vp, _vp, _i, _i, _i, _vp],
    'asr_beam_step_wide': [ctypes.POINTER(BeamStep), _vp, _sz, _vp],
    'asr_beam_attend': [ctypes.POINTER(BeamAttend), _vp],
    'asr_ctc_prefix_init_batched': [_vp, _vp, _vp, _i, _i, _i, _i, _vp],
    'asr_ctc_prefix_score_batched': [_vp, _vp, _vp, _vp, _vp, _vp, _vp, _vp, _i, _i, _i, _i, _i, _vp],
    'asr_ctc_beam_search': [_vp, _vp, _i, _i, _i, _i, _i, _i, _vp, _vp, _vp, _vp, _vp, _sz, _vp],
    'asr_ctc_beam_lm_init': [_i, _i, _i, _vp, _sz, _vp],
    'asr_ctc_beam_lm_advance': [_vp, _vp, _vp, _i, _i, _i, _i, _i, _f, _f, _i, _vp, _vp, _vp, _vp, _vp, _vp, _sz, _vp],
    'asr_ctc_beam_lm_readout': [_i, _i, _i, _i, _vp, _vp, _vp, _vp, _vp, _vp, _sz, _vp],
    'asr_rescore_pack': [_vp, _vp, _vp, _vp, _i, _i, _i, _i, _i, _vp, _vp, _vp, _vp, _vp, _vp],
    'asr_rescore_nbest': [_vp, _l, _l, _vp, _l, _vp, _vp, _vp, _vp, _i, _i, _i, _i, _f, _vp, _vp, _vp, _vp],
    'asr_rescore_lm_input': [_vp, _l, _i, _i, ctypes.c_int64, _vp, _vp],
    'asr_rescore_token_logp': [_vp, _l, _l, _vp, _l, _vp, _i, _i, _i, _vp, _l, _vp],
    'asr_rescore_rank_lm': [_vp, _vp, _vp, _l, _vp, _vp, _i, _i, _i, _f, _f, _f, _vp, _vp, _vp, _vp],
    'asr_ctc_align': [_vp, _vp, _vp, _vp, _i, _i, _i, _i, _vp, _vp, _vp, _vp, _vp, _vp, _vp, _vp, _sz, _vp],
    'asr_ragged_align': [_vp, _vp, _vp, _i, _i, _i, _i, _i, _vp],
    'asr_ragged_unalign': [_vp, _l, _l, _vp, _vp, _i, _i, _i, _i, _i, _i, _i, _i, _vp],
    'asr_ragged_zero_tail': [_vp, _vp, _i, _i, _i, _i, _i, _i, _vp],
    'asr_gemm16': [_vp, _vp, _vp, _vp, _i, _i, _i, _l, _l, _l, _i, _i, _i, _i, _i, _i, _i, _i, _i, _i, _vp],
    'asr_lstm16_fwd': [_vp, _vp, _vp, _vp, _i, _i, _i, _i, _vp, _sz, ctypes.c_uint, _i, _vp],
    'asr_lstm16_bwd': [_vp, _vp, _vp, _vp, _i, _i, _i, _i, _vp, _sz, ctypes.c_uint, _i, _vp],
    'asr_cast_bf16': [_vp, _vp, _l, _vp],
    'asr_cast_f32': [_vp, _vp, _l, _i, _vp],
    'asr_rnn_pack_weights': [_vp, _vp, _vp, _vp, _vp, _vp, _vp, _vp, _vp, _i, _i, _i, _i, _vp],
    'asr_dropout_downsample16_fwd': [_vp, _l, _l, _vp, _i, _i, _i, _i, _i, _i, _f, _u64, _vp],
    'asr_dropout_downsample16_bwd': [_vp, _vp, _i, _i, _i, _i, _i, _i, _f, _u64, _vp],
    'asr_act_bwd16': [_vp, _vp, _vp, _l, _i, _vp],
    'asr_colsum16': [_vp, _l, _i, _i, _vp, _vp, _i, _vp],
    'asr_debug_occupy': [_i, _i, ctypes.c_double, _vp],
    'asr_scrub_workspace': [_vp, _sz, _vp, _vp],
    'asr_stream_create_cu_mask': [_i, _i, ctypes.POINTER(_vp)],
    'asr_stream_destroy': [_vp],
}
_RESTYPES = {
    'asr_last_error': (ctypes.c_char_p, []),
    'asr_device_arch': (ctypes.c_char_p, []),
    'asr_version': (ctypes.c_int, []),
    'asr_lstm_workspace_bytes': (_sz, [_i, _i, _i]),
    'asr_gru_rec_workspace_bytes': (_sz, [_i, _i]),
    'asr_specaug_workspace_bytes': (_sz, [_i]),
    'asr_cmvn_workspace_bytes': (_sz, [_i, _i]),
    'asr_specaug_policy_workspace_bytes': (_sz, [_i]),
    'asr_wave_augment_workspace_bytes': (_sz, [_i, _i, _i]),
    'asr_lstm_set_persistent': (ctypes.c_int, [_i]),
    'asr_lstm_plan': (ctypes.c_int, [_i, _i, _i, _i, _i]),
    'asr_gemm_plan': (ctypes.c_int, [_vp, _vp, _vp, _vp, _i, _i, _i, _l, _l, _l, _i, _i, _i, _i, _i, _i, _l, _l, _l, _i, _i, _i, _P(_i)]),
    'asr_conv3x3_plan': (ctypes.c_int, [_vp, _vp, _vp, _vp, _i, _i, _i, _i, _i, _i, _i, _i, _i, _P(_i)]),
    'asr_gemm16_route': (ctypes.c_int, [_vp, _vp, _vp, _vp, _i, _i, _i, _l, _l, _l, _i, _i, _i, _i, _i, _i, _i, _i, _i, _i]),
    'asr_gemm16_plan': (ctypes.c_int, [_vp, _vp, _vp, _vp, _i, _i, _i, _l, _l, _l, _i, _i, _i, _i, _i, _i, _i, _i, _i, _i, _P(_i)]),
    'asr_lstm16_workspace_bytes': (_sz, [_i, _i, _i, _i]),
    'asr_lstm16_set_bwd_form': (ctypes.c_int, [_i]),
    'asr_lstm16_bwd_form': (ctypes.c_int, [_i, _i, _i]),
    'asr_ctc_loss_workspace_bytes': (_sz, [_i, _i, _i]),
    'asr_beam_step_wide_workspace_bytes': (_sz, [_i, _i]),
    'asr_ctc_beam_search_workspace_bytes': (_sz, [_i, _i, _i]),
    'asr_ctc_beam_lm_workspace_bytes': (_sz, [_i, _i, _i]),
    'asr_ctc_align_workspace_bytes': (_sz, [_i, _i, _i]),
    'asr_fbank_workspace_bytes': (_sz, [_i, _i, _i, _i]),
    'asr_att_decoder_bwd_workspace_bytes': (_sz, [_P(DecDims)]),
    'asr_att_decoder_fwd_work_bytes': (_sz, [_P(DecDims)]),
    'asr_att_decoder_set_persistent': (ctypes.c_int, [_i]),
    'asr_att_decoder_bwd_status_offset': (_sz, [_P(DecDims)]),
    'asr_att_decoder_bwd_persistent_tiles': (ctypes.c_int, [_P(DecDims)]),
    'asr_att_decoder_fwd_plan': (ctypes.c_int, [_P(DecDims)]),
    'asr_att_decoder_bwd_plan': (ctypes.c_int, [_P(DecDims)]),
    'asr_beam_attend_resident_max_t': (ctypes.c_int, [_i]),
}


class HipLibraryMissing(RuntimeError):
    pass


def _load():
    if not os.path.exists(LIB_PATH):
        raise HipLibraryMissing(
            'libasr_hip.so not found at %s — build it with `python -c "import __graft_entry__ as g; g.build()"` '
            '(there is no CPU fallback for the HIP path)' % LIB_PATH)
    lib = ctypes.CDLL(LIB_PATH)
    for name, argtypes in SIGNATURES.items():
        fn = getattr(lib, name)
        fn.argtypes = argtypes
        fn.restype = ctypes.c_int
    for name, (rt, at) in _RESTYPES.items():
        fn = getattr(lib, name)
        fn.argtypes = at
        fn.restype = rt
    return lib


_lib = _load()


def lib():
    return _lib


def exported_symbols():
    return list(SIGNATURES.keys()) + list(_RESTYPES.keys())


def stream_ptr():
    return ctypes.c_void_p(torch.cuda.current_stream().cuda_stream)


_watch = {}
_status = {}


def status_word(device=None):
    dev = torch.cuda.current_device() if device is None else torch.device(device).index
    if dev not in _status:
        _status[dev] = torch.zeros(1, dtype=torch.int32, device='cuda:%d' % dev)
    return _status[dev]


def watch_abort(t, offset=0, release=False):
    if t is None:
        return
    lst = _watch.setdefault(t.device.index, [])
    lst.append((t, t.data_ptr() + int(offset), release))
    if len(lst) >= 32:
        collect_status()


def abort_guard(t, offset=0):
    if t is None:
        return
    addr = t.data_ptr() + int(offset)
    for _, a, _r in _watch.get(t.device.index, ()):
        if a == addr:
            collect_status()
            return


def collect_status():
    dev = torch.cuda.current_device()
    lst = _watch.get(dev)
    st = status_word(dev)
    while lst:
        chunk, lst[:] = lst[:32], lst[32:]
        arr = (_vp * len(chunk))(*[a for _, a, _r in chunk])
        call('asr_status_collect', arr, len(chunk), ptr(st), stream_ptr())
        for t, _, rel in chunk:
            if rel:
                handoff_release(t)
    return st
# ... 257 lines not shown
    del _side['keep'][:]


def ptr(t):
    if t is None:
        return None
    if not t.is_cuda:
        raise RuntimeError('HIP path got a non-CUDA tensor; there is no CPU fallback')
    if t.device.index != torch.cuda.current_device():
        raise RuntimeError('tensor on cuda:%d but the current device is cuda:%d: the HIP kernels launch on the current '
                           'device (call torch.cuda.set_device first)' % (t.device.index, torch.cuda.current_device()))
    return ctypes.c_void_p(t.data_ptr())


def check(rc, what):
    if rc != 0:
        raise RuntimeError('%s failed (%d): %s' % (what, rc, _lib.asr_last_error().decode()))


def call(name, *args):
    check(getattr(_lib, name)(*args), name)


def _f32c(t):
    assert t.dtype == torch.float32, t.dtype
    return t


def gemm(A, B, C, M, N, K, lda, ldb, ldc, a_kc=1, b_kc=1, bias=None, act=ACT_NONE, accum=0, splits=1,
         batch=1, sA=0, sB=0, sC=0, seqT=0, bshift=0, prec=BF16):
    call('asr_gemm', ptr(_f32c(A)), ptr(_f32c(B)), ptr(_f32c(C)), ptr(bias), M, N, K, lda, ldb, ldc,
         a_kc, b_kc, act, accum, splits, batch, sA, sB, sC, seqT, bshift, prec, stream_ptr())


def gemm16(A, B, C, M, N, K, lda, ldb, ldc, a_kc=1, b_kc=1, bias=None, act=ACT_NONE, accum=0, splits=1, perm_h=0,
           seqT=0, bshift=0, b_time_padded=0, a_off=0, b_off=0):
    assert A.dtype == torch.bfloat16 and B.dtype == torch.bfloat16 and C.dtype in (torch.bfloat16, torch.float32)
    pa = ctypes.c_void_p(ptr(A).value + 2 * a_off)
    pb = ctypes.c_void_p(ptr(B).value + 2 * b_off)
    call('asr_gemm16', pa, pb, ptr(C), ptr(bias), M, N, K, lda, ldb, ldc, a_kc, b_kc, act, accum, splits,
         1 if C.dtype == torch.bfloat16 else 0, perm_h, seqT, bshift, b_time_padded, stream_ptr())


def wgrad_splits(rows, out_rows=None, out_cols=None):
    if out_rows is None:
        return max(1, min(32, rows // 1024))
    tiles = ((out_rows + 127) // 128) * ((out_cols + 127) // 128)
    return max(1, min(64, rows // 512, int(round(900.0 / tiles))))


def linear_fwd(x2d, W, b, out2d, act=ACT_NONE, prec=BF16):
    M, K = x2d.shape
    N = W.shape[0]
    gemm(x2d, W, out2d, M, N, K, x2d.stride(0), W.stride(0), out2d.stride(0), 1, 1, bias=b, act=act, prec=prec)


def linear_bwd(x2d, W, dy2d, dW, db, dx2d=None, prec=BF16, accum_dx=0):
    M, K = x2d.shape
    N = W.shape[0]
    gemm(dy2d, x2d, dW, N, K, M, dy2d.stride(0), x2d.stride(0), dW.stride(0), 0, 0, accum=1, splits=wgrad_splits(M, N, K), prec=prec)
    if db is not None:
        call('asr_colsum', ptr(dy2d), dy2d.stride(0), M, N, ptr(db), stream_ptr())
    if dx2d is not None:
        gemm(dy2d, W, dx2d, M, K, N, dy2d.stride(0), W.stride(0), dx2d.stride(0), 1, 0, accum=accum_dx, prec=prec)


def linear_bwd_input(W, dy2d, dx2d, prec=BF16, accum_dx=0):
    M, N = dy2d.shape
    K = W.shape[1]
    gemm(dy2d, W, dx2d, M, K, N, dy2d.stride(0), W.stride(0), dx2d.stride(0), 1, 0, accum=accum_dx, prec=prec)


def dec_weights_struct(tensors, nl):
    w = DecWeights()
    for n in _DEC_W_FIELDS + ['Wc', 'bc']:
        setattr(w, n, tensors[n].data_ptr())
    for n in ('Wih', 'Whh', 'bih', 'bhh'):
        arr = getattr(w, n)
        for l in range(nl):
            arr[l] = tensors[n][l].data_ptr()
    return w


def dec_state_struct(tensors):
    s = DecState()
    for n, _ in DecState._fields_:
        if n == 'work_bytes':
            w = tensors.get('work')
            s.work_bytes = int(w.numel() * w.element_size()) if w is not None else 0
            continue
        t = tensors.get(n)
        setattr(s, n, t.data_ptr() if t is not None else None)
    return s
```

### e2e-asr-pytorch_amd/src/step.py

```python
import torch


def train_step(model, optimizer, ctc_crit, att_crit, feat, feat_len, txt, decode_step, tf_rate=1.0, dp=None,
               clip=5.0, txt_len=None, optimize=True, emb_decoder=None, emb_optimizer=None):
    from src import hipabi as H
    cur = torch.cuda.current_stream()
    if not (feat.is_cuda and H.step_overlaps(dp)) or cur != torch.cuda.default_stream():
        return _train_step(model, optimizer, ctc_crit, att_crit, feat, feat_len, txt, decode_step, tf_rate, dp, clip, txt_len, optimize,
                           emb_decoder, emb_optimizer)
    with H.on_work_stream():
        out = _train_step(model, optimizer, ctc_crit, att_crit, feat, feat_len, txt, decode_step, tf_rate, dp, clip, txt_len, optimize,
                          emb_decoder, emb_optimizer)
    for v in out.values():
        if torch.is_tensor(v):
            v.record_stream(cur)
    return out


def step_emb_optimizer(emb_optimizer, model_normsq, grad_mul=1.0):
    eo = emb_optimizer.opt if hasattr(emb_optimizer, 'opt') else emb_optimizer
    eo.normsq = model_normsq
    eo.step(clip=0.0, grad_mul=grad_mul, use_norm=True)


def scale_weight(w_dev, k):
    from src import hipabi as H
    from src.functions import loss_weight
    if not torch.is_tensor(w_dev):
        return loss_weight(float(w_dev) * k, torch.device('cuda', torch.cuda.current_device()))
    w = w_dev.reshape(1).to(torch.float32).contiguous()
    out = torch.empty(1, dtype=torch.float32, device=w.device)
    H.call('asr_loss_mix', H.ptr(w), H.ptr(loss_weight(k, w.device)), None, None, H.ptr(out), H.stream_ptr())
    return out


def _train_step(model, optimizer, ctc_crit, att_crit, feat, feat_len, txt, decode_step, tf_rate=1.0, dp=None,
                clip=5.0, txt_len=None, optimize=True, emb_decoder=None, emb_optimizer=None):
    opt = optimizer.opt if hasattr(optimizer, 'opt') else optimizer
    opt.zero_grad()
    if txt_len is None:
        txt_len = torch.sum(txt != 0, dim=-1)
    if emb_decoder is not None:
        emb_decoder.zero_grad()
    out = forward_losses(model, ctc_crit, att_crit, feat, feat_len, txt, decode_step, tf_rate, dp, txt_len, emb_decoder)
    normsq, grad_mul = backward_update(out['total_loss'], opt, dp, clip, optimize, emb_optimizer)
    out.update(total_loss=out['total_loss'].detach(), grad_normsq=normsq, grad_mul=grad_mul)
    return out


def forward_losses(model, ctc_crit, att_crit, feat, feat_len, txt, decode_step, tf_rate, dp, txt_len, emb_decoder=None):
    from src import hipabi as H
    if emb_decoder is None:
        ctc_output, encode_len, att_output, att_align, _ = model(feat, feat_len, decode_step, tf_rate=tf_rate, teacher=txt, ctc_async=True)
        emb_loss = None
    else:
        if getattr(emb_decoder, 'apply_fuse', False) and tf_rate != 1:
            raise ValueError('embedding fusion cannot be combined with scheduled sampling (tf_rate = %r < 1): the fused output is a '
                             'log-probability, which the reference hands to Categorical as logits and fails' % (tf_rate,))
        ctc_output, encode_len, att_output, att_align, dec_state = model(feat, feat_len, decode_step, tf_rate=tf_rate, teacher=txt,
                                                                         ctc_async=True, get_dec_state=True)
        emb_loss, fuse_output = emb_decoder(dec_state, att_output, label=txt[:, :att_output.shape[1]])
        if fuse_output is not None:
            att_output = fuse_output
    total, ctc_loss, att_loss = None, None, None
    from src.functions import LossMixFn, loss_weight
    dev = feat.device
    if ctc_output is not None:
        if getattr(ctc_output, '_asr_side', False):
            with H.side_branch(False, txt, txt_len):
                ctc_loss = ctc_crit(ctc_output.transpose(0, 1), txt, encode_len, txt_len)
            H.join_branch(ctc_loss, ctc_output)
        else:
            ctc_loss = ctc_crit(ctc_output.transpose(0, 1), txt, encode_len, txt_len)
    w_att = None
    if att_output is not None:
        b, t, _ = att_output.shape
        att_loss = att_crit(att_output.view(b * t, -1), txt[:, :t].reshape(-1))
        if dp is not None and dp.world > 1:
            w_att = scale_weight(dp.ce_weight(txt_len.sum()), 1 - model.ctc_weight)
        else:
            w_att = loss_weight(1 - model.ctc_weight, dev)
    if ctc_loss is not None and att_loss is not None:
        total = LossMixFn.apply(ctc_loss, loss_weight(model.ctc_weight, dev), att_loss, w_att)
    elif ctc_loss is not None:
        total = LossMixFn.apply(ctc_loss, loss_weight(model.ctc_weight, dev), None, None)
    else:
        total = LossMixFn.apply(att_loss, w_att, None, None)
    if emb_loss is not None:
        total = LossMixFn.apply(total, loss_weight(1.0, dev), emb_loss, loss_weight(emb_decoder.weight, dev))
    return {'total_loss': total, 'ctc_loss': ctc_loss, 'att_loss': att_loss, 'emb_loss': emb_loss, 'ctc_output': ctc_output,
            'att_output': att_output, 'att_align': att_align, 'encode_len': encode_len}


def backward_update(total, opt, dp=None, clip=5.0, optimize=True, emb_optimizer=None):
    from src import hipabi as H
    total.backward()
    H.join_side()
    grad_mul = 1.0
    if dp is not None:
        dp.finish()
        grad_mul = dp.grad_mul
    normsq = opt.grad_norm()
    if optimize:
        opt.step(clip=clip, grad_mul=grad_mul, use_norm=True)
        if emb_optimizer is not None:
            step_emb_optimizer(emb_optimizer, normsq, grad_mul)
    return normsq, grad_mul
```

### e2e-asr-pytorch_amd/src/util.py

```python
import math
import time

import torch
from torch import nn

from src import functions as F_hip


def init_weights_(model):
    for p in model.parameters():
        d = p.data
        if d.dim() == 1:
            d.zero_()
        elif d.dim() == 2:
            d.normal_(0, 1.0 / math.sqrt(d.size(1)))
        elif d.dim() in (3, 4):
            n = d.size(1)
            for k in d.size()[2:]:
                n *= k
            d.normal_(0, 1.0 / math.sqrt(n))
        else:
            raise NotImplementedError


def init_gate_(bias):
    n = bias.size(0)
    bias.data[n // 4:n // 2].fill_(1.)
    return bias


class CTCLoss(nn.Module):

    def __init__(self, blank=0, zero_infinity=False):
        super().__init__()
        assert blank == 0 and not zero_infinity

    def forward(self, log_probs_tbv, targets, input_lengths, target_lengths):
        if not torch.is_tensor(input_lengths):
            input_lengths = torch.as_tensor(input_lengths)
        if not torch.is_tensor(target_lengths):
            target_lengths = torch.as_tensor(target_lengths)
        return F_hip.CTCLossFn.apply(log_probs_tbv.transpose(0, 1), targets, input_lengths, target_lengths)


class CrossEntropyLoss(nn.Module):

    def __init__(self, ignore_index=0):
        super().__init__()
        assert ignore_index == 0

    def forward(self, logits, target):
        return F_hip.SeqLossFn.apply(logits, target, 0, logits.shape[-1], 0.0)


class LabelSmoothingLoss(nn.Module):

    def __init__(self, classes, smoothing=0.0, dim=-1):
        super().__init__()
        self.cls, self.smoothing = classes, smoothing

    def forward(self, pred, target):
        return F_hip.SeqLossFn.apply(pred, target, 1, self.cls, float(self.smoothing))


class Timer():

    def __init__(self):
        self.prev_t = time.time()
        self.clear()

    def set(self):
        self.prev_t = time.time()

    def cnt(self, mode):
        self.time_table[mode] += time.time() - self.prev_t
        self.set()
        if mode == 'bw':
            self.click += 1

    def show(self):
        total = sum(self.time_table.values())
        n = max(self.click, 1)
        msg = '{:.3f} sec/step (rd {:.1f}% | fw {:.1f}% | bw {:.1f}%)'.format(
            total / n, *[100 * self.time_table[k] / max(total, 1e-9) for k in ('rd', 'fw', 'bw')])
        self.clear()
        return msg

    def clear(self):
        self.time_table = {'rd': 0, 'fw': 0, 'bw': 0}
        self.click = 0


def human_format(num):
    magnitude = 0
    while num >= 1000:
        magnitude += 1
        num /= 1000.0
    return '{:3.1f}{}'.format(num, [' ', 'K', 'M', 'G', 'T', 'P'][magnitude])


def edit_distance(a, b):
    if len(a) < len(b):
        a, b = b, a
    prev = list(range(len(b) + 1))
    for i, x in enumerate(a, 1):
        cur = [i]
        for j, y in enumerate(b, 1):
            cur.append(min(prev[j] + 1, cur[j - 1] + 1, prev[j - 1] + (x != y)))
        prev = cur
    return prev[-1]


def cal_er(tokenizer, pred, truth, mode='wer', ctc=False):
    if pred is None:
        return float('nan')
    if len(pred.shape) >= 3:
        pred = pred.argmax(dim=-1)
    er = []
    for p, t in zip(pred.tolist(), truth.tolist()):
        p = tokenizer.decode(p, ignore_repeat=ctc)
        t = tokenizer.decode(t)
        if mode in ('wer', 'per'):
            p, t = p.split(' '), t.split(' ')
        er.append(1. if len(t) == 0 else float(edit_distance(p, t)) / len(t))
    return sum(er) / len(er)
# ... 39 lines not shown
```

### include/asr_hip.h

```cpp
#ifndef ASR_HIP_H
#define ASR_HIP_H
#include <stdint.h>
#include <stddef.h>

#ifdef __cplusplus
extern "C" {
#endif

#define ASR_OK 0
#define ASR_E_ARG (-1)
#define ASR_E_LAUNCH (-2)
#define ASR_E_UNSUPPORTED (-3)

#define ASR_F32 0
#define ASR_BF16 1

#define ASR_ACT_NONE 0
#define ASR_ACT_TANH 1
#define ASR_ACT_RELU 2

typedef void* asr_stream_t;

const char* asr_last_error(void);
int asr_version(void);
const char* asr_device_arch(void);

int asr_gemm(const float* A, const float* B, float* C, const float* bias,
             int M, int N, int K, long lda, long ldb, long ldc,
             int a_kc, int b_kc, int act, int accum, int splits,
             int batch, long sA, long sB, long sC, int seqT, int bshift,
             int prec, asr_stream_t stream);
int asr_gemm_plan(const float* A, const float* B, float* C, const float* bias,
                  int M, int N, int K, long lda, long ldb, long ldc,
                  int a_kc, int b_kc, int act, int accum, int splits,
                  int batch, long sA, long sB, long sC, int seqT, int bshift,
                  int prec, int out[8]);

size_t asr_lstm_workspace_bytes(int B, int H, int ND);
int asr_lstm_set_persistent(int on);
int asr_lstm_plan(int B, int T, int H, int ND, int prec);
int asr_lstm_fwd(float* gates, const float* whh, const float* bias2, float* y, float* c,
                 int B, int T, int H, int ND, int prec,
                 void* workspace, size_t workspace_bytes, asr_stream_t stream);
int asr_lstm_bwd(float* gates, const float* whh, const float* dy, const float* c,
                 int B, int T, int H, int ND, int prec,
                 void* workspace, size_t workspace_bytes, asr_stream_t stream);

size_t asr_lstm16_workspace_bytes(int B, int H, int ND, int backward);
int asr_lstm16_fwd(void* gates16, const float* whh, void* y16, float* c, int B, int T, int H, int ND,
                   void* workspace, size_t workspace_bytes, unsigned epoch, int reserved_cus, asr_stream_t stream);
int asr_lstm16_bwd(void* gates16, const float* whh, const void* dy16, const float* c, int B, int T, int H, int ND,
                   void* workspace, size_t workspace_bytes, unsigned epoch, int reserved_cus, asr_stream_t stream);
int asr_lstm16_set_bwd_form(int form);
int asr_lstm16_bwd_form(int B, int H, int ND);
int asr_gemm16(const void* A, const void* B, void* C, const float* bias, int M, int N, int K, long lda, long ldb, long ldc,
               int a_kc, int b_kc, int act, int accum, int splits, int c_bf16, int perm_h,
               int seqT, int bshift, int b_time_padded, asr_stream_t stream);
int asr_gemm16_route(const void* A, const void* B, void* C, const float* bias, int M, int N, int K, long lda, long ldb, long ldc,
                     int a_kc, int b_kc, int act, int accum, int splits, int c_bf16, int perm_h,
                     int seqT, int bshift, int b_time_padded);
int asr_gemm16_plan(const void* A, const void* B, void* C, const float* bias, int M, int N, int K, long lda, long ldb, long ldc,
                    int a_kc, int b_kc, int act, int accum, int splits, int c_bf16, int perm_h,
                    int seqT, int bshift, int b_time_padded, int out[8]);
int asr_rnn_pack_weights(const float* w_ih, const float* b_ih, const float* b_hh, const float* pj,
                         void* w_ih16, void* w_ihT16, float* bias, void* pj16, void* pjT16,
                         int H, int ND, int Din, int D, asr_stream_t stream);
int asr_cast_bf16(const float* src, void* dst, long n, asr_stream_t stream);
int asr_cast_f32(const void* src, float* dst, long n, int accum, asr_stream_t stream);
int asr_dropout_downsample16_fwd(const void* y, long y_bstride, long y_off, void* z, int B, int T, int D, int T2, int rate,
                                 int style, float p, uint64_t seed, asr_stream_t stream);
int asr_dropout_downsample16_bwd(const void* dz, void* dy, int B, int T, int D, int T2, int rate, int style,
                                 float p, uint64_t seed, asr_stream_t stream);
int asr_act_bwd16(const void* dout, const void* out, void* dpre, long n, int act, asr_stream_t stream);
int asr_colsum16(const void* A, long lda, int M, int N, float* out, float* out2, int perm_h, asr_stream_t stream);

int asr_dropout_downsample_fwd(const float* y, float* z, int B, int T, int D, int T2, int rate, int style,
                               float p, uint64_t seed, asr_stream_t stream);
int asr_dropout_downsample_bwd(const float* dz, float* dy, int B, int T, int D, int T2, int rate, int style,
                               float p, uint64_t seed, asr_stream_t stream);
int asr_dropout_mask(float* mask, long n, float p, uint64_t seed, asr_stream_t stream);

int asr_ragged_align(const void* src, void* dst, const int64_t* lens, int B, int T, int ND, int W, int elem_bytes,
                     asr_stream_t stream);
int asr_ragged_unalign(const void* src, long src_bstride, long src_off, void* dst, const int64_t* lens, int B, int T,
                       int ND, int H, int T2, int rate, int style, int elem_bytes, asr_stream_t stream);
int asr_ragged_zero_tail(void* buf, const int64_t* lens, int B, int T, int Ttot, int t_off, int W, int elem_bytes,
                         asr_stream_t stream);

int asr_act_bwd(const float* dout, const float* out, float* dpre, long n, int act, asr_stream_t stream);
int asr_colsum(const float* A, long lda, int M, int N, float* out, asr_stream_t stream);
int asr_colsum2(const float* A, long lda, int M, int N, float* out, float* out2, asr_stream_t stream);
int asr_log_softmax(const float* x, float* out, long rows, int V, asr_stream_t stream);
int asr_logsoftmax_relu_bwd(const float* dlogp, const float* logp, const float* act, float* dpre,
                            long rows, int V, asr_stream_t stream);
int asr_layernorm_fwd(const float* x, const float* w, const float* b, float* y, float* stats,
                      long rows, int n, float eps, int relu, asr_stream_t stream);
int asr_layernorm_bwd(const float* dy, const float* x, const float* w, const float* b, const float* stats,
                      float* dx, float* dw, float* db, long rows, int n, int relu, asr_stream_t stream);

size_t asr_ctc_loss_workspace_bytes(int B, int T, int L);
int asr_ctc_loss(const float* logp, const int64_t* targets, const int64_t* input_len, const int64_t* target_len,
                 float* nll, float* loss, float* grad, int B, int T, int V, int L, float gscale,
                 void* workspace, size_t workspace_bytes, asr_stream_t stream);

int asr_xent(const float* logits, const int64_t* targets, long target_ld, float* dlogits, float* loss,
             float* accum2, int B, int L, int V, int mode, int classes, float smoothing, float gscale,
             asr_stream_t stream);

#define ASR_MAX_DEC_LAYERS 4
typedef struct {
    int B, Tp, E;
    int A, Q;
    int Dd, NL, V;
    int Kn, Ks;
    int L;
    float temperature;
} asr_dec_dims_t;

typedef struct {
    const float *Wq, *bq;
    const float *Wk, *bk;
    const float *Wconv;
    const float *Wproj;
    const float *wg, *bg;
    const float *emb;
    const float *Wih[ASR_MAX_DEC_LAYERS], *Whh[ASR_MAX_DEC_LAYERS];
    const float *bih[ASR_MAX_DEC_LAYERS], *bhh[ASR_MAX_DEC_LAYERS];
    const float *Wc, *bc;
} asr_dec_weights_t;

typedef struct {
    float *Wq, *bq, *Wk, *bk, *Wconv, *Wproj, *wg, *bg, *emb;
    float *Wih[ASR_MAX_DEC_LAYERS], *Whh[ASR_MAX_DEC_LAYERS], *bih[ASR_MAX_DEC_LAYERS], *bhh[ASR_MAX_DEC_LAYERS];
    float *Wc, *bc;
} asr_dec_grads_t;

typedef struct {
    float* key;
    float* att;
    float* q;
    float* xin;
    float* gates;
    float* cs;
    float* hs;
    float* logits;
    float* energy;
    float* conv;
    void* key16;
    void* enc16;
    void* work;
    size_t work_bytes;
    int64_t* tokens;
} asr_dec_state_t;

int asr_att_decoder_fwd(const asr_dec_dims_t* dims, const asr_dec_weights_t* weights,
                        const float* enc, const int64_t* enc_len, const int64_t* teacher, int teacher_ld,
                        const asr_dec_state_t* state, int prec, asr_stream_t stream);
size_t asr_att_decoder_bwd_workspace_bytes(const asr_dec_dims_t* dims);
int asr_att_decoder_set_persistent(int flags);
int asr_att_decoder_fwd_plan(const asr_dec_dims_t* dims);
int asr_att_decoder_bwd_plan(const asr_dec_dims_t* dims);
int asr_att_decoder_energy_plan(const asr_dec_dims_t* dims, int* knmax, int* tpw);
int asr_att_decoder_bwd_persistent_tiles(const asr_dec_dims_t* dims);
size_t asr_att_decoder_bwd_status_offset(const asr_dec_dims_t* dims);
size_t asr_att_decoder_fwd_work_bytes(const asr_dec_dims_t* dims);
int asr_att_decoder_bwd(const asr_dec_dims_t* dims, const asr_dec_weights_t* weights, const asr_dec_grads_t* grads,
                        const float* enc, const int64_t* enc_len, const asr_dec_state_t* state,
                        const float* dlogits, float* denc,
                        void* workspace, size_t workspace_bytes, int prec, asr_stream_t stream);

int asr_att_decoder_bwd_ex(const asr_dec_dims_t* dims, const asr_dec_weights_t* weights, const asr_dec_grads_t* grads,
                           const float* enc, const int64_t* enc_len, const asr_dec_state_t* state,
                           const float* dlogits, float* denc,
                           void* workspace, size_t workspace_bytes, int prec, int defer_params, int* looped_out,
                           asr_stream_t stream);
int asr_att_decoder_bwd_params(const asr_dec_dims_t* dims, const asr_dec_weights_t* weights, const asr_dec_grads_t* grads,
                               const float* enc, const int64_t* enc_len, const asr_dec_state_t* state, const float* dlogits,
                               void* workspace, size_t workspace_bytes, int looped, int prec, asr_stream_t stream);
int asr_att_decoder_bwd_hs(const asr_dec_dims_t* dims, const asr_dec_weights_t* weights, const asr_dec_grads_t* grads,
                           const float* enc, const int64_t* enc_len, const asr_dec_state_t* state,
                           const float* dlogits, const float* dhs_ext, float* denc,
                           void* workspace, size_t workspace_bytes, int prec, int defer_params, int* looped_out,
                           asr_stream_t stream);

int asr_emb_cos_loss(const float* x, const float* table, const int64_t* label, long label_ld, float* loss, float* dx, float* dy,
                     float* row_loss, int B, int L, int E, int V, asr_stream_t stream);
int asr_emb_fuse_fwd(const float* dec_logit, long dec_ld, const float* emb_logit, const float* temp, int temp_stride,
                     const float* lam, int lam_stride, int lam_sigmoid, float* out, float* stats, int64_t* argmax, long argmax_ld,
                     int N, int V, asr_stream_t stream);
int asr_emb_fuse_bwd(const float* dout, const float* dec_logit, long dec_ld, const float* emb_logit, const float* temp,
                     int temp_stride, const float* lam, int lam_stride, int lam_sigmoid, const float* stats, float* d_dec_logit,
                     float* d_emb_logit, float* d_temp, float* d_lam_raw, float* work, int N, int V, asr_stream_t stream);
int asr_row_normalize_fwd(const float* x, float* y, long N, int E, asr_stream_t stream);
int asr_row_normalize_bwd(const float* dy, const float* x, float* dx, long N, int E, asr_stream_t stream);

int asr_sumsq(const float* x, long n, double* out, asr_stream_t stream);
int asr_scale(float* x, long n, float k, asr_stream_t stream);
int asr_scale_dev(const float* in, float* out, long n, const float* alpha, asr_stream_t stream);
int asr_loss_mix(const float* a, const float* wa, const float* b, const float* wb, float* out, asr_stream_t stream);
int asr_status_collect(const void* const* abort_words, int n, unsigned* status, asr_stream_t stream);
int asr_adadelta_step(float* param, const float* grad, float* square_avg, float* acc_delta, long n,
                      float lr, float rho, float eps, float weight_decay, float clip,
                      const double* normsq, float grad_mul, const unsigned* status, asr_stream_t stream);
int asr_adam_step(float* param, const float* grad, float* exp_avg, float* exp_avg_sq, float* max_exp_avg_sq, long n,
                  float lr, float beta1, float beta2, float eps, float weight_decay, int step, float clip,
                  const double* normsq, float grad_mul, const unsigned* status, unsigned long long* step_counter, asr_stream_t stream);
int asr_embedding_bwd(const float* dy, long dy_ld, const int64_t* idx, float* demb, int rows, int width, int V, asr_stream_t stream);

size_t asr_fbank_workspace_bytes(int B, int T, int win, int n_fft);
int asr_fbank(const float* wav, const int64_t* wav_len, float* out, const float* dft_table, const float* mel_fb,
              const float* window, int B, int N, int T, int win, int hop, int n_fft, int nmel,
              float preemph, float ref_db, float min_db,
              void* workspace, size_t workspace_bytes, asr_stream_t stream);
int asr_delta_stack(const float* x, const int64_t* lens, float* out, const float* filters,
                    int B, int T, int F, int channels, int taps, asr_stream_t stream);
int asr_specaug(float* x, const int64_t* lens, const int* draws_in, int* draws_out, int B, int T, int D,
                int time_width, int freq_width, uint64_t seed, asr_stream_t stream);
size_t asr_specaug_workspace_bytes(int B);
int asr_specaug_ws(float* x, const int64_t* lens, const int* draws_in, int* draws_out, int B, int T, int D,
                   int time_width, int freq_width, uint64_t seed, void* workspace, size_t workspace_bytes, asr_stream_t stream);
size_t asr_cmvn_workspace_bytes(int B, int D);
int asr_cmvn(float* x, const int64_t* lens, float* stats_out , int B, int T, int D, float eps,
             void* workspace, size_t workspace_bytes, asr_stream_t stream);

size_t asr_specaug_policy_workspace_bytes(int B);
int asr_specaug_policy(const float* x, const int64_t* lens, float* out, const int* draws_in, int* draws_out,
                       int B, int T, int D, int warp, int freq_masks, int freq_width, int time_masks, int time_width,
                       int time_ratio_pm, int time_count_pm, int fill , uint64_t seed,
                       void* workspace, size_t workspace_bytes, asr_stream_t stream);

int asr_wave_draws(const int64_t* wav_len, const float* draws_in, float* draws_out, float* rates_out, int B, int N, int n_fft,
                   uint64_t seed, asr_stream_t stream);
int asr_wave_noise(float* wav, const int64_t* wav_len, const float* draws, int B, int N, uint64_t seed, asr_stream_t stream);
int asr_wave_stft(const float* wav, const int64_t* wav_len, const float* rates, int rate_stride, const float* table, float* spec,
                  int B, int N, int n_fft, asr_stream_t stream);
int asr_wave_pvoc(const float* spec, const int64_t* wav_len, const float* rates, int rate_stride, float* out, int B, int N,
                  int n_fft, asr_stream_t stream);
int asr_wave_istft(const float* out_spec, const int64_t* wav_len, const float* rates, int rate_stride, const float* table,
                   float* dst, long dst_stride, int keep_len, int B, int N, int n_fft, asr_stream_t stream);
int asr_wave_resample(const float* src, long src_stride, const int64_t* wav_len, const float* rates, int rate_stride, float* wav,
                      int B, int N, int n_fft, asr_stream_t stream);
size_t asr_wave_augment_workspace_bytes(int B, int N, int n_fft);
int asr_wave_augment(float* wav, const int64_t* wav_len, const float* draws_in, float* draws_out, const float* table, int B,
// ... 160 lines not shown
```

Baseline: 1.149 million frames/s.

## Run CTC loss sweeps as extra roles inside the persistent attention decoder forward kernel

Moves the CTC forward/backward lattice sweep and gradient work into spare workgroups of the persistent attention-decoder forward kernel through a CTC job struct passed in the decoder state. The CTC device code moves into a shared header so both the standalone kernels and the decoder can use it. The aim is to overlap the serial CTC recurrence with the decoder's own serial loop and to save the separate launches. In exchange it adds a lot of plumbing, a 'ran' flag with a version check and a fallback path, and risks contention for CUs and LDS with the decoder.

```diff
diff --git a/e2e-asr-pytorch_amd/csrc/ctc.hip b/e2e-asr-pytorch_amd/csrc/ctc.hip
--- a/e2e-asr-pytorch_amd/csrc/ctc.hip
+++ b/e2e-asr-pytorch_amd/csrc/ctc.hip
@@ -1,166 +1,37 @@
-#include "common.h"
+#include "ctc_body.h"
 
 namespace {
 
-struct CtcP {
-    const float* lp;
-    const int64_t* tgt;
-    const int64_t* in_len;
-    const int64_t* tgt_len;
-    float* nll;
-    float* loss;
-    float* grad;
-    float* alpha;
-    float* beta;
-    int B, T, V, L, Smax;
-    float gscale;
-};
-
-__device__ __forceinline__ float lse2(float a, float b) {
-    const float m = fmaxf(a, b);
-    if (m == -INFINITY) return -INFINITY;
-    return m + __logf(1.f + __expf(-fabsf(a - b)));
-}
-
-__device__ __forceinline__ float lse3(float a, float b, float c) {
-    const float m = fmaxf(fmaxf(a, b), c);
-    if (m == -INFINITY) return -INFINITY;
-    const float md = __builtin_amdgcn_fmed3f(a, b, c), mn = fminf(fminf(a, b), c);
-    return m + __logf(1.f + __expf(md - m) + __expf(mn - m));
-}
-
-constexpr int CTC_FCH = 8;
-constexpr size_t CTC_GRAD_LDS = 60 * 1024;
-
 __global__ __launch_bounds__(1024) void ctc_sweep_kernel(CtcP p, int CF) {
     extern __shared__ __attribute__((aligned(16))) unsigned char smem[];
-    const int b = blockIdx.x, back = blockIdx.y;
-    const int tid = threadIdx.x, NTH = blockDim.x;
-    const int V = p.V, T = p.T;
-    int tl = (int)p.tgt_len[b];
-    tl = max(0, min(tl, p.L));
-    const int S = 2 * tl + 1;
-    int Tin = (int)p.in_len[b];
-    Tin = max(0, min(Tin, T));
-    int* ext = reinterpret_cast<int*>(smem);
-    float* buf0 = reinterpret_cast<float*>(ext + p.Smax + 2) + 2;
-    float* buf1 = buf0 + p.Smax + 6;
-    float* s_lp = buf1 + p.Smax + 4;
-    const float* lp = p.lp + (long)b * T * V;
-    float* lat = (back ? p.beta : p.alpha) + (long)b * T * p.Smax;
-
-    for (int s = tid; s < p.Smax + 2; s += NTH) ext[s] = (s < S && (s & 1)) ? (int)p.tgt[(long)b * p.L + (s >> 1)] : 0;
-    for (int s = tid - 2; s < p.Smax + 2; s += NTH) { buf0[s] = -INFINITY; buf1[s] = -INFINITY; }
-    __syncthreads();
-    if (Tin == 0) {
-        if (!back && tid == 0) {
-            const float n = (tl == 0) ? 0.f : INFINITY;
-            p.nll[b] = n;
-        }
-        return;
-    }
-    const int nwb = (p.L + 1 + 63) >> 6;
-    const bool label = (tid >> 6) >= nwb;
-    const int s = label ? 2 * (tid - 64 * nwb) + 1 : 2 * tid;
-    const bool sok = s < S;
-    const int sr = sok ? s : 0;
-    const int e = sok ? ext[s] : 0;
-    bool skip = false;
-    if (sok && !back) skip = (s >= 2) && e != 0 && e != ext[s - 2];
-    if (sok && back) skip = (s + 2 < S) && ext[s + 2] != 0 && ext[s + 2] != e;
-    float* prev = buf0;
-    float* cur = buf1;
-    for (int c0 = 0; c0 < Tin; c0 += CF) {
-        const int nf = min(CF, Tin - c0);
-        const int tlo = back ? Tin - c0 - nf : c0;
-        __syncthreads();
-        for (int i = tid; i < nf * V; i += NTH) s_lp[i] = lp[(long)tlo * V + i];
-        __syncthreads();
-        for (int i = 0; i < nf; ++i) {
-            const int t = back ? Tin - 1 - (c0 + i) : c0 + i;
-            const float lpe = s_lp[(t - tlo) * V + e];
-            float a;
-            if (c0 + i == 0) {
-                if (!back) a = (s == 0 || s == 1) ? lpe : -INFINITY;
-                else       a = (s == S - 1 || s == S - 2) ? lpe : -INFINITY;
-            } else {
-                const int d1 = back ? 1 : -1;
-                if (label) a = lse3(prev[sr], prev[sr + d1], skip ? prev[sr + 2 * d1] : -INFINITY);
-                else       a = lse2(prev[sr], prev[sr + d1]);
-                a += lpe;
-            }
-            if (sok) { cur[s] = a; lat[(long)t * p.Smax + s] = a; }
-            __syncthreads();
-            float* tmp = prev; prev = cur; cur = tmp;
-        }
-    }
-    if (!back && tid == 0) {
-        float ll = prev[S - 1];
-        if (S > 1) ll = lse2(ll, prev[S - 2]);
-        p.nll[b] = -ll;
-    }
+    ctc_sweep_body(p, CF, blockIdx.x, blockIdx.y, threadIdx.x, blockDim.x, smem);
 }
 
 template <int FCH>
 __global__ __launch_bounds__(1024) void ctc_grad_kernel(CtcP p) {
     extern __shared__ __attribute__((aligned(16))) unsigned char smem[];
-    const int b = blockIdx.y, t0 = blockIdx.x * FCH;
-    const int tid = threadIdx.x, NTH = blockDim.x, lane = tid & 63, wave = tid >> 6, nwave = NTH >> 6;
-    const int V = p.V, T = p.T;
-    int tl = (int)p.tgt_len[b];
-    tl = max(0, min(tl, p.L));
-    const int S = 2 * tl + 1;
-    int Tin = (int)p.in_len[b];
-    Tin = max(0, min(Tin, T));
-    float* acc = reinterpret_cast<float*>(smem);
-    float* blk = acc + FCH * V;
-    const float* lp = p.lp + (long)b * T * V;
-    float* grad = p.grad + (long)b * T * V;
-    for (int i = tid; i < FCH * V; i += NTH) acc[i] = 0.f;
-    const int s = tid;
-    const bool sok = s < S;
-    const int e = (sok && (s & 1)) ? (int)p.tgt[(long)b * p.L + (s >> 1)] : 0;
-    const float nll = p.nll[b];
-    const float scale = p.gscale / (float)(max(tl, 1) * p.B);
-    if (blockIdx.x == 0 && blockIdx.y == 0 && tid == 0) {
-        float sum = 0.f;
-        for (int bb = 0; bb < p.B; ++bb) {
-            int l = (int)p.tgt_len[bb];
-            l = max(1, min(l, p.L));
-            sum += p.nll[bb] / (float)(l * p.B);
-        }
-        *p.loss = sum;
-    }
-    float occ[FCH];
-#pragma unroll
-    for (int f = 0; f < FCH; ++f) {
-        const int t = t0 + f;
-        occ[f] = 0.f;
-        if (sok && t < Tin) {
-            const long li = ((long)b * T + t) * p.Smax + s;
-            occ[f] = expf(p.alpha[li] + p.beta[li] - lp[(long)t * V + e] + nll);
-        }
-    }
-    __syncthreads();
-#pragma unroll
-    for (int f = 0; f < FCH; ++f) {
-        if (sok && (s & 1) && t0 + f < Tin) atomicAdd(&acc[f * V + e], occ[f]);
-        const float bsum = wave_sum((sok && !(s & 1)) ? occ[f] : 0.f);
-        if (lane == 0) blk[f * nwave + wave] = bsum;
-    }
-    __syncthreads();
-    for (int i = tid; i < FCH * V; i += NTH) {
-        const int f = i / V, v = i - f * V, t = t0 + f;
-        if (t >= T) continue;
-        float g = 0.f;
-        if (t < Tin) {
-            float a = acc[i];
-            if (v == 0) for (int w = 0; w < nwave; ++w) a += blk[f * nwave + w];
-            if (!(nll < INFINITY)) a = NAN;
-            g = scale * (expf(lp[(long)t * V + v]) - a);
-        }
-        grad[(long)t * V + v] = g;
-    }
+    if (blockIdx.x == 0 && blockIdx.y == 0 && threadIdx.x == 0) ctc_mean_loss(p);
+    ctc_grad_body<FCH>(p, blockIdx.y, blockIdx.x * FCH, threadIdx.x, blockDim.x, smem);
+}
+
+struct CtcLaunch { int nthr, CF, fch; size_t lds_s, lds_g1; };
+int ctc_launch_plan(int T, int V, int L, CtcLaunch* k) {
+    const int Smax = 2 * L + 1;
+    ASR_REQUIRE(Smax <= 1024, ASR_E_UNSUPPORTED, "asr_ctc_loss: 2L+1=%d states exceed one workgroup", Smax);
+    const int nthr = 64 * ((L + 1 + 63) / 64 + (L + 63) / 64);
+    const size_t fixed = (size_t)(Smax + 2) * 4 + 2 * (size_t)(Smax + 6) * 4 + 16;
+    int CF = (int)((60 * 1024 - fixed) / ((size_t)V * 4));
+    ASR_REQUIRE(CF >= 1, ASR_E_UNSUPPORTED, "asr_ctc_loss: V=%d classes exceed the LDS budget: at most V=%d with 2L+1=%d states "
+                "(one frame of log-probs beside the lattice buffers in 60 KB)", V, (int)((60 * 1024 - fixed) / 4), Smax);
+    if (CF > T) CF = T;
+    const size_t lds_s = fixed + (size_t)CF * V * 4;
+    const size_t lds_g1 = (size_t)(V + nthr / 64) * 4;
+    ASR_REQUIRE(lds_g1 <= CTC_GRAD_LDS, ASR_E_UNSUPPORTED, "asr_ctc_loss: V=%d classes exceed the %zu bytes of LDS of the gradient kernel",
+                V, CTC_GRAD_LDS);
+    int fch = CTC_FCH;
+    while ((size_t)fch * lds_g1 > CTC_GRAD_LDS) fch >>= 1;
+    *k = CtcLaunch{nthr, CF, fch, lds_s, lds_g1};
+    return ASR_OK;
 }
 
 }
@@ -178,19 +49,11 @@
     const int Smax = 2 * L + 1;
     float* wsf = (float*)workspace;
     CtcP p{logp, targets, input_len, target_len, nll, loss, grad, wsf, wsf + (size_t)B * T * Smax, B, T, V, L, Smax, gscale};
-    ASR_REQUIRE(Smax <= 1024, ASR_E_UNSUPPORTED, "asr_ctc_loss: 2L+1=%d states exceed one workgroup", Smax);
-    const int nthr = 64 * ((L + 1 + 63) / 64 + (L + 63) / 64);
-    const size_t fixed = (size_t)(Smax + 2) * 4 + 2 * (size_t)(Smax + 6) * 4 + 16;
-    int CF = (int)((60 * 1024 - fixed) / ((size_t)V * 4));
-    ASR_REQUIRE(CF >= 1, ASR_E_UNSUPPORTED, "asr_ctc_loss: V=%d classes exceed the LDS budget: at most V=%d with 2L+1=%d states "
-                "(one frame of log-probs beside the lattice buffers in 60 KB)", V, (int)((60 * 1024 - fixed) / 4), Smax);
-    if (CF > T) CF = T;
-    const size_t lds_s = fixed + (size_t)CF * V * 4;
-    const size_t lds_g1 = (size_t)(V + nthr / 64) * 4;
-    ASR_REQUIRE(lds_g1 <= CTC_GRAD_LDS, ASR_E_UNSUPPORTED, "asr_ctc_loss: V=%d classes exceed the %zu bytes of LDS of the gradient kernel",
-                V, CTC_GRAD_LDS);
-    int fch = CTC_FCH;
-    while ((size_t)fch * lds_g1 > CTC_GRAD_LDS) fch >>= 1;
+    CtcLaunch k;
+    const int rc = ctc_launch_plan(T, V, L, &k);
+    if (rc != ASR_OK) return rc;
+    const int nthr = k.nthr, CF = k.CF, fch = k.fch;
+    const size_t lds_s = k.lds_s, lds_g1 = k.lds_g1;
     hipStream_t st = (hipStream_t)stream;
     hipLaunchKernelGGL(ctc_sweep_kernel, dim3(B, 2), dim3(nthr), lds_s, st, p, CF);
     const dim3 gg(cdiv(T, fch), B);
@@ -203,3 +66,14 @@
     ASR_LAUNCH_CHECK("asr_ctc_loss");
     return ASR_OK;
 }
+
+extern "C" int asr_ctc_loss_launch_plan(int B, int T, int V, int L, long long* out) {
+    ASR_REQUIRE(out, ASR_E_ARG, "asr_ctc_loss_launch_plan: null pointer");
+    ASR_REQUIRE(B > 0 && T > 0 && V > 1 && L > 0, ASR_E_ARG, "asr_ctc_loss_launch_plan: bad dims");
+    CtcLaunch k;
+    const int rc = ctc_launch_plan(T, V, L, &k);
+    if (rc != ASR_OK) return rc;
+    out[0] = B; out[1] = 2; out[2] = k.nthr; out[3] = (long long)k.lds_s; out[4] = k.CF;
+    out[5] = cdiv(T, k.fch); out[6] = B; out[7] = (long long)(k.fch * k.lds_g1);
+    return ASR_OK;
+}
diff --git a/e2e-asr-pytorch_amd/csrc/ctc_body.h b/e2e-asr-pytorch_amd/csrc/ctc_body.h
--- /dev/null
+++ b/e2e-asr-pytorch_amd/csrc/ctc_body.h
@@ -0,0 +1,225 @@
+#pragma once
+#include "common.h"
+#include <algorithm>
+
+namespace {
+
+struct CtcP {
+    const float* lp;
+    const int64_t* tgt;
+    const int64_t* in_len;
+    const int64_t* tgt_len;
+    float* nll;
+    float* loss;
+    float* grad;
+    float* alpha;
+    float* beta;
+    int B, T, V, L, Smax;
+    float gscale;
+};
+
+__device__ __forceinline__ float lse2(float a, float b) {
+    const float m = fmaxf(a, b);
+    if (m == -INFINITY) return -INFINITY;
+    return m + __logf(1.f + __expf(-fabsf(a - b)));
+}
+
+__device__ __forceinline__ float lse3(float a, float b, float c) {
+    const float m = fmaxf(fmaxf(a, b), c);
+    if (m == -INFINITY) return -INFINITY;
+    const float md = __builtin_amdgcn_fmed3f(a, b, c), mn = fminf(fminf(a, b), c);
+    return m + __logf(1.f + __expf(md - m) + __expf(mn - m));
+}
+
+constexpr int CTC_FCH = 8;
+constexpr size_t CTC_GRAD_LDS = 60 * 1024;
+
+__host__ __device__ inline int ctc_sweep_threads(int L) { return 64 * ((L + 1 + 63) / 64 + (L + 63) / 64); }
+__host__ __device__ inline size_t ctc_sweep_fixed(int Smax) { return (size_t)(Smax + 2) * 4 + 2 * (size_t)(Smax + 6) * 4 + 16; }
+
+__device__ __forceinline__ void ctc_sweep_body(const CtcP& p, int CF, int b, int back, int tid, int NTH, unsigned char* smem) {
+    const int V = p.V, T = p.T;
+    int tl = (int)p.tgt_len[b];
+    tl = max(0, min(tl, p.L));
+    const int S = 2 * tl + 1;
+    int Tin = (int)p.in_len[b];
+    Tin = max(0, min(Tin, T));
+    int* ext = reinterpret_cast<int*>(smem);
+    float* buf0 = reinterpret_cast<float*>(ext + p.Smax + 2) + 2;
+    float* buf1 = buf0 + p.Smax + 6;
+    float* s_lp = buf1 + p.Smax + 4;
+    const float* lp = p.lp + (long)b * T * V;
+    float* lat = (back ? p.beta : p.alpha) + (long)b * T * p.Smax;
+
+    for (int s = tid; s < p.Smax + 2; s += NTH) ext[s] = (s < S && (s & 1)) ? (int)p.tgt[(long)b * p.L + (s >> 1)] : 0;
+    for (int s = tid - 2; s < p.Smax + 2; s += NTH) { buf0[s] = -INFINITY; buf1[s] = -INFINITY; }
+    __syncthreads();
+    if (Tin == 0) {
+        if (!back && tid == 0) {
+            const float n = (tl == 0) ? 0.f : INFINITY;
+            p.nll[b] = n;
+        }
+        return;
+    }
+    const int nwb = (p.L + 1 + 63) >> 6;
+    const bool label = (tid >> 6) >= nwb;
+    const int s = label ? 2 * (tid - 64 * nwb) + 1 : 2 * tid;
+    const bool sok = s < S;
+    const int sr = sok ? s : 0;
+    const int e = sok ? ext[s] : 0;
+    bool skip = false;
+    if (sok && !back) skip = (s >= 2) && e != 0 && e != ext[s - 2];
+    if (sok && back) skip = (s + 2 < S) && ext[s + 2] != 0 && ext[s + 2] != e;
+    float* prev = buf0;
+    float* cur = buf1;
+    for (int c0 = 0; c0 < Tin; c0 += CF) {
+        const int nf = min(CF, Tin - c0);
+        const int tlo = back ? Tin - c0 - nf : c0;
+        __syncthreads();
+        for (int i = tid; i < nf * V; i += NTH) s_lp[i] = lp[(long)tlo * V + i];
+        __syncthreads();
+        for (int i = 0; i < nf; ++i) {
+            const int t = back ? Tin - 1 - (c0 + i) : c0 + i;
+            const float lpe = s_lp[(t - tlo) * V + e];
+            float a;
+            if (c0 + i == 0) {
+                if (!back) a = (s == 0 || s == 1) ? lpe : -INFINITY;
+                else       a = (s == S - 1 || s == S - 2) ? lpe : -INFINITY;
+            } else {
+                const int d1 = back ? 1 : -1;
+                if (label) a = lse3(prev[sr], prev[sr + d1], skip ? prev[sr + 2 * d1] : -INFINITY);
+                else       a = lse2(prev[sr], prev[sr + d1]);
+                a += lpe;
+            }
+            if (sok) { cur[s] = a; lat[(long)t * p.Smax + s] = a; }
+            __syncthreads();
+            float* tmp = prev; prev = cur; cur = tmp;
+        }
+    }
+    if (!back && tid == 0) {
+        float ll = prev[S - 1];
+        if (S > 1) ll = lse2(ll, prev[S - 2]);
+        p.nll[b] = -ll;
+    }
+}
+
+__device__ __forceinline__ void ctc_mean_loss(const CtcP& p) {
+    float sum = 0.f;
+    for (int bb = 0; bb < p.B; ++bb) {
+        int l = (int)p.tgt_len[bb];
+        l = max(1, min(l, p.L));
+        sum += p.nll[bb] / (float)(l * p.B);
+    }
+    *p.loss = sum;
+}
+
+template <int FCH, bool FIX = false>
+__device__ __forceinline__ void ctc_grad_body(const CtcP& p, int b, int t0, int tid, int NTH, unsigned char* smem) {
+    const int lane = tid & 63, wave = tid >> 6, nwave = NTH >> 6;
+    const int V = p.V, T = p.T;
+    int tl = (int)p.tgt_len[b];
+    tl = max(0, min(tl, p.L));
+    const int S = 2 * tl + 1;
+    int Tin = (int)p.in_len[b];
+    Tin = max(0, min(Tin, T));
+    float* acc = reinterpret_cast<float*>(smem);
+    unsigned long long* acc64 = reinterpret_cast<unsigned long long*>(smem);
+    float* blk = acc + (FIX ? 2 : 1) * FCH * V;
+    const float* lp = p.lp + (long)b * T * V;
+    float* grad = p.grad + (long)b * T * V;
+    if constexpr (FIX) { for (int i = tid; i < FCH * V; i += NTH) acc64[i] = 0ull; }
+    else { for (int i = tid; i < FCH * V; i += NTH) acc[i] = 0.f; }
+    const int s = tid;
+    const bool sok = s < S;
+    const int e = (sok && (s & 1)) ? (int)p.tgt[(long)b * p.L + (s >> 1)] : 0;
+    const float nll = p.nll[b];
+    const float scale = p.gscale / (float)(max(tl, 1) * p.B);
+    float occ[FCH];
+#pragma unroll
+    for (int f = 0; f < FCH; ++f) {
+        const int t = t0 + f;
+        occ[f] = 0.f;
+        if (sok && t < Tin) {
+            const long li = ((long)b * T + t) * p.Smax + s;
+            occ[f] = expf(p.alpha[li] + p.beta[li] - lp[(long)t * V + e] + nll);
+        }
+    }
+    __syncthreads();
+#pragma unroll
+    for (int f = 0; f < FCH; ++f) {
+        if (sok && (s & 1) && t0 + f < Tin) {
+            if constexpr (FIX) atomicAdd(&acc64[f * V + e], (unsigned long long)__float2ll_rn(occ[f] * 1099511627776.f));
+            else atomicAdd(&acc[f * V + e], occ[f]);
+        }
+        const float bsum = wave_sum((sok && !(s & 1)) ? occ[f] : 0.f);
+        if (lane == 0) blk[f * nwave + wave] = bsum;
+    }
+    __syncthreads();
+    for (int i = tid; i < FCH * V; i += NTH) {
+        const int f = i / V, v = i - f * V, t = t0 + f;
+        if (t >= T) continue;
+        float g = 0.f;
+        if (t < Tin) {
+            float a = FIX ? (float)((double)(long long)acc64[i] * (1.0 / 1099511627776.0)) : acc[i];
+            if (v == 0) for (int w = 0; w < nwave; ++w) a += blk[f * nwave + w];
+            if (!(nll < INFINITY)) a = NAN;
+            g = scale * (expf(lp[(long)t * V + v]) - a);
+        }
+        grad[(long)t * V + v] = g;
+    }
+}
+
+struct CtcRolePlan { int R, side, CF, fch; unsigned area; };
+struct CtcRole { CtcP p; CtcRolePlan pl; };
+
+inline CtcRolePlan ctc_role_plan(int B, int T, int V, int L, int block, size_t lds, int spare) {
+    const CtcRolePlan none{0, 0, 0, 0, 0u};
+    if (B < 1 || T < 1 || V < 2 || L < 1 || spare < 1) return none;
+    const int Smax = 2 * L + 1, nthr = ctc_sweep_threads(L);
+    CtcRolePlan pl{std::min(B, spare), 0, 0, CTC_FCH, 0u};
+    if (2 * nthr <= block) pl.side = 1;
+    else if (nthr > block) return none;
+    const size_t fixed = ctc_sweep_fixed(Smax), per = (pl.side ? lds / 2 : lds) & ~(size_t)15;
+    if (per < fixed + (size_t)V * 4) return none;
+    pl.CF = (int)std::min<size_t>((per - fixed) / ((size_t)V * 4), (size_t)T);
+    pl.area = (unsigned)per;
+    const size_t lds_g1 = (size_t)(2 * V + block / 64) * 4;
+    if (lds_g1 > lds) return none;
+    while ((size_t)pl.fch * lds_g1 > std::min(lds, CTC_GRAD_LDS)) pl.fch >>= 1;
+    return pl;
+}
+
+__device__ __forceinline__ void ctc_role_run(const CtcRole& c, int r, unsigned* arrive, unsigned char* smem) {
+    const CtcP& p = c.p;
+    const int tid = threadIdx.x, NTH = blockDim.x;
+    for (int b = r; b < p.B; b += c.pl.R) {
+        __syncthreads();
+        if (c.pl.side) {
+            const int half = NTH >> 1, back = tid >= half ? 1 : 0;
+            ctc_sweep_body(p, c.pl.CF, b, back, tid - back * half, half, smem + (size_t)back * c.pl.area);
+        } else {
+            ctc_sweep_body(p, c.pl.CF, b, 0, tid, NTH, smem);
+            __syncthreads();
+            ctc_sweep_body(p, c.pl.CF, b, 1, tid, NTH, smem);
+        }
+        for (int t0 = 0; t0 < p.T; t0 += c.pl.fch) {
+            __syncthreads();
+            switch (c.pl.fch) {
+                case 8: ctc_grad_body<8, true>(p, b, t0, tid, NTH, smem); break;
+                case 4: ctc_grad_body<4, true>(p, b, t0, tid, NTH, smem); break;
+                case 2: ctc_grad_body<2, true>(p, b, t0, tid, NTH, smem); break;
+                default: ctc_grad_body<1, true>(p, b, t0, tid, NTH, smem); break;
+            }
+        }
+    }
+    if (tid == 0) {
+        __threadfence();
+        const unsigned n = atomicAdd(arrive, 1u);
+        if (n == (unsigned)c.pl.R - 1u) {
+            __threadfence();
+            ctc_mean_loss(p);
+        }
+    }
+}
+
+}
diff --git a/e2e-asr-pytorch_amd/csrc/decoder.hip b/e2e-asr-pytorch_amd/csrc/decoder.hip
--- a/e2e-asr-pytorch_amd/csrc/decoder.hip
+++ b/e2e-asr-pytorch_amd/csrc/decoder.hip
@@ -1152,6 +1152,12 @@
 }
 extern "C" int asr_att_decoder_fwd_plan(const asr_dec_dims_t* dims) { return dims ? dec_fwd_plan_info(*dims).kind : 0; }
 extern "C" int asr_att_decoder_bwd_plan(const asr_dec_dims_t* dims) { return dims ? dec_bwd_plan_info(*dims).kind : 0; }
+extern "C" int asr_att_decoder_fwd_ctc_roles(const asr_dec_dims_t* dims, int T, int L_ctc, int V, int* plan) {
+    int pl[4] = {0, 0, 0, 0};
+    if (dims && T > 0 && L_ctc > 0 && V > 1 && check_dims(*dims, "asr_att_decoder_fwd_ctc_roles") == ASR_OK) dec_fwd_ctc_roles(*dims, T, L_ctc, V, pl);
+    if (plan) for (int i = 0; i < 4; ++i) plan[i] = pl[i];
+    return pl[0];
+}
 extern "C" int asr_att_decoder_energy_plan(const asr_dec_dims_t* dims, int* knmax, int* tpw) {
     ASR_REQUIRE(dims && knmax && tpw, ASR_E_ARG, "asr_att_decoder_energy_plan: null pointer");
     const int rc = check_dims(*dims, "asr_att_decoder_energy_plan");
@@ -1174,6 +1180,15 @@
     int rc = check_dims(d, "asr_att_decoder_fwd");
     if (rc != ASR_OK) return rc;
     hipStream_t st = (hipStream_t)stream;
+    asr_dec_state_t sv = *state;
+    if (asr_ctc_job_t* job = sv.ctc_job) {
+        job->ran = 0;
+        const bool ok = job->logp && job->targets && job->input_len && job->target_len && job->nll && job->loss && job->grad &&
+                        job->workspace && job->B == d.B && job->T > 0 && job->V > 1 && job->L > 0 && 2 * job->L + 1 <= 1024 &&
+                        job->workspace_bytes >= asr_ctc_loss_workspace_bytes(job->B, job->T, job->L);
+        if (!ok) sv.ctc_job = nullptr;
+    }
+    state = &sv;
     DecP p{d, *weights, *state, enc, enc_len};
     const bool bf = (prec == ASR_BF16);
     if (state->work && state->work_bytes >= 256)
diff --git a/e2e-asr-pytorch_amd/csrc/decoder_cluster.h b/e2e-asr-pytorch_amd/csrc/decoder_cluster.h
--- a/e2e-asr-pytorch_amd/csrc/decoder_cluster.h
+++ b/e2e-asr-pytorch_amd/csrc/decoder_cluster.h
@@ -2,6 +2,7 @@
 #include "common.h"
 #include "handoff.h"
 #include "decoder_internal.h"
+#include "ctc_body.h"
 #include <stdlib.h>
 #include <algorithm>
 
@@ -105,6 +106,8 @@
     int KC, KCP;
     int allow_local;
     unsigned epoch;
+    int cluster_wgs;
+    CtcRole ctc;
 };
 
 struct ConvGeo { int NKS, WKP, IMG_LD, need; };
@@ -258,6 +261,7 @@
 
 constexpr int EPOCH_WORD = 1008;
 constexpr size_t STATUS_CLEAR_BYTES = 4032;
+constexpr int CTC_ARRIVE_WORD = 1000;
 __global__ void bump_epoch_kernel(unsigned* status) { status[EPOCH_WORD] = status[EPOCH_WORD] + 1u; status[DEC_FWD_LAUNCHED_WORD] = 1u; }
 __global__ void clear_work_kernel(uint4* work, long n16) {
     for (long i = blockIdx.x * (long)blockDim.x + threadIdx.x; i < n16; i += (long)gridDim.x * blockDim.x)
diff --git a/e2e-asr-pytorch_amd/csrc/decoder_internal.h b/e2e-asr-pytorch_amd/csrc/decoder_internal.h
--- a/e2e-asr-pytorch_amd/csrc/decoder_internal.h
+++ b/e2e-asr-pytorch_amd/csrc/decoder_internal.h
@@ -12,6 +12,7 @@
 DecPlanInfo dec_bwd_plan_info(const asr_dec_dims_t& d);
 int dec_fwd_persistent(const asr_dec_dims_t& d, const asr_dec_weights_t& w, const asr_dec_state_t& s, const float* enc,
                        const int64_t* enc_len, void* work, size_t work_bytes, hipStream_t st);
+void dec_fwd_ctc_roles(const asr_dec_dims_t& d, int T, int L_ctc, int V, int* plan);
 constexpr int DEC_FWD_LAUNCHED_WORD = 1009;
 constexpr size_t DEC_STATUS_BYTES = 4096;
 int dec_bwd_persistent(const asr_dec_dims_t& d, const asr_dec_weights_t& w, const asr_dec_state_t& s, const int64_t* enc_len,
diff --git a/e2e-asr-pytorch_amd/csrc/decoder_persist.hip b/e2e-asr-pytorch_amd/csrc/decoder_persist.hip
--- a/e2e-asr-pytorch_amd/csrc/decoder_persist.hip
+++ b/e2e-asr-pytorch_amd/csrc/decoder_persist.hip
@@ -9,7 +9,14 @@
     g_persist_fwd = flags & 1; g_persist_bwd = (flags >> 1) & 1; g_stream_fwd = (flags >> 2) & 1; g_stream_bwd = (flags >> 3) & 1;
     return old;
 }
+static int g_ctc_roles = -2;
+extern "C" int asr_att_decoder_set_ctc_roles(int cap) {
+    const int old = g_ctc_roles == -2 ? (env_switch("ASR_DEC_CTC_ROLE", 0) ? -1 : 0) : g_ctc_roles;
+    g_ctc_roles = cap < 0 ? -1 : cap;
+    return old;
+}
 static void read_switches() {
+    if (g_ctc_roles == -2) g_ctc_roles = env_switch("ASR_DEC_CTC_ROLE", 0) ? -1 : 0;
     if (g_persist_fwd < 0) g_persist_fwd = env_switch("ASR_DEC_PERSIST", 1);
     if (g_persist_bwd < 0) g_persist_bwd = env_switch("ASR_DEC_PERSIST_BWD", 1);
     if (g_stream_fwd < 0) g_stream_fwd = env_switch("ASR_DEC_STREAM", 0);
@@ -27,6 +34,21 @@
     read_switches();
     const BwdPlan r = persist_plan_b(d), s = stream_plan_b(d), pl = chosen_plan(r, s, g_stream_bwd);
     return {pl.kind, pl.NT, std::max(r.NT, s.NT), std::max(r.total, s.total)};
+}
+static CtcRolePlan fwd_ctc_role(const asr_dec_dims_t& d, const FwdPlan& pl, int T, int V, int L_ctc) {
+    read_switches();
+    if (pl.kind != 1 || g_ctc_roles == 0) return CtcRolePlan{};
+    int dev = 0, cus = 0;
+    if (hipGetDevice(&dev) != hipSuccess || hipDeviceGetAttribute(&cus, hipDeviceAttributeMultiprocessorCount, dev) != hipSuccess) return CtcRolePlan{};
+    int spare = cus - (int)cluster_grid(d, pl.NT).x;
+    if (g_ctc_roles > 0) spare = std::min(spare, g_ctc_roles);
+    return ctc_role_plan(d.B, T, V, L_ctc, 64 * (NCW + NPW), pl.lds, spare);
+}
+void dec_fwd_ctc_roles(const asr_dec_dims_t& d, int T, int L_ctc, int V, int* plan) {
+    read_switches();
+    if (!g_persist_fwd) return;
+    const CtcRolePlan r = fwd_ctc_role(d, fwd_plan(d), T, V, L_ctc);
+    plan[0] = r.R; plan[1] = r.side; plan[2] = r.CF; plan[3] = r.fch;
 }
 float* dec_bwd_dgates(const asr_dec_dims_t& d, void* work) { return bwd_work(d, bwd_plan(d), work).dgates; }
 
@@ -50,6 +72,7 @@
     return 2 * shorts + 4 * floats;
 }
 
+
 template <int KNMAX, int TPW>
 __global__ __launch_bounds__(64 * (NCW + NPW)) void dec_fwd_persist(PD p) {
     constexpr int TE = 8 * TPW;
@@ -60,6 +83,7 @@
     __shared__ float s_scale[NCW][32];
     const asr_dec_dims_t& d = p.d;
     const int id = blockIdx.x, xcd = id & 7, slot = id >> 3;
+    if (id >= p.cluster_wgs) { ctc_role_run(p.ctc, id - p.cluster_wgs, p.status + CTC_ARRIVE_WORD, smem); return; }
     const int cb = slot / p.NT, j = slot - cb * p.NT;
     const int b = cb * 8 + xcd;
     if (b >= d.B) return;
@@ -318,19 +342,33 @@
     embproj.prec = ASR_BF16;
     int rc = gemm_run(embproj, st);
     if (rc != ASR_OK) return rc;
-    const PD p{d, w, s, enc, enc_len, wk.wcat16, wk.embproj, wk.xbuf, wk.status, pl.NT, pl.TE, pl.UPW, pl.QPW, pl.CPW, pl.HG2, pl.QG2, pl.SG2, pl.KC,
-               pl.KCP, xcd_local_allowed()};
-    const ClusterLaunch go{"asr_att_decoder_fwd(persistent)", 160 * 1024 - 2048, cluster_grid(d, pl.NT), dim3(64 * (NCW + NPW)), pl.lds, st};
+    PD p{d, w, s, enc, enc_len, wk.wcat16, wk.embproj, wk.xbuf, wk.status, pl.NT, pl.TE, pl.UPW, pl.QPW, pl.CPW, pl.HG2, pl.QG2, pl.SG2, pl.KC,
+         pl.KCP, xcd_local_allowed()};
+    dim3 grid = cluster_grid(d, pl.NT);
+    p.cluster_wgs = (int)grid.x;
+    asr_ctc_job_t* job = s.ctc_job;
+    if (job) {
+        const int Smax = 2 * job->L + 1;
+        float* wsf = (float*)job->workspace;
+        p.ctc.p = CtcP{job->logp, job->targets, job->input_len, job->target_len, job->nll, job->loss, job->grad, wsf,
+                       wsf + (size_t)job->B * job->T * Smax, job->B, job->T, job->V, job->L, Smax, job->gscale};
+        p.ctc.pl = fwd_ctc_role(d, pl, job->T, job->V, job->L);
+        grid.x += p.ctc.pl.R;
+        if (!p.ctc.pl.R) job = nullptr;
+    }
+    const ClusterLaunch go{"asr_att_decoder_fwd(persistent)", 160 * 1024 - 2048, grid, dim3(64 * (NCW + NPW)), pl.lds, st};
+    rc = 1;
     if (d.Kn <= 4) {
-        if (pl.tpw == 2) return go.run<dec_fwd_persist<4, 2>>(p);
-        if (pl.tpw == 4) return go.run<dec_fwd_persist<4, 4>>(p);
-        if (pl.tpw == 5) return go.run<dec_fwd_persist<4, 5>>(p);
-        return go.run<dec_fwd_persist<4, 8>>(p);
-    }
-    if (pl.tpw == 2) return go.run<dec_fwd_persist<10, 2>>(p);
-    if (pl.tpw == 4) return go.run<dec_fwd_persist<10, 4>>(p);
-    if (pl.tpw == 5) return go.run<dec_fwd_persist<10, 5>>(p);
-    return 1;
+        if (pl.tpw == 2) rc = go.run<dec_fwd_persist<4, 2>>(p);
+        else if (pl.tpw == 4) rc = go.run<dec_fwd_persist<4, 4>>(p);
+        else if (pl.tpw == 5) rc = go.run<dec_fwd_persist<4, 5>>(p);
+        else rc = go.run<dec_fwd_persist<4, 8>>(p);
+    }
+    else if (pl.tpw == 2) rc = go.run<dec_fwd_persist<10, 2>>(p);
+    else if (pl.tpw == 4) rc = go.run<dec_fwd_persist<10, 4>>(p);
+    else if (pl.tpw == 5) rc = go.run<dec_fwd_persist<10, 5>>(p);
+    if (rc == ASR_OK && job) job->ran = 1;
+    return rc;
 }
 
 namespace {
diff --git a/e2e-asr-pytorch_amd/src/asr.py b/e2e-asr-pytorch_amd/src/asr.py
--- a/e2e-asr-pytorch_amd/src/asr.py
+++ b/e2e-asr-pytorch_amd/src/asr.py
@@ -245,7 +245,7 @@
         return msg
 
     def forward(self, audio_feature, feature_len, decode_step, tf_rate=0.0, teacher=None,
-                emb_decoder=None, get_dec_state=False, get_logit=False, ctc_async=False):
+                emb_decoder=None, get_dec_state=False, get_logit=False, ctc_async=False, ctc_target=None):
         if not audio_feature.is_cuda:
             raise RuntimeError('ASR (HIP path) needs CUDA tensors; there is no CPU fallback')
         fuse_dec = (emb_decoder if emb_decoder is not None and getattr(emb_decoder, 'enable', False) and emb_decoder.apply_fuse
@@ -284,8 +284,14 @@
                 att_seq, hs = st['att'].view(d.B, 1, d.L, d.Tp), st['hs']
                 self._last_tokens = st['tokens']
             else:
+                ctc = None
+                if (ctc_target is not None and ctc_output is not None and not side_ctc and dp is None and self.training
+                        and torch.is_grad_enabled() and teacher is not None and float(tf_rate) == 1.0 and not get_logit):
+                    ctc = {'logp': ctc_output, 'targets': ctc_target[0], 'input_len': encode_len, 'target_len': ctc_target[1]}
                 att_output, att_seq, hs = F_hip.AttDecoderFn.apply(ctx.anchor, encode_feature, encode_len, teacher, L, self, self.prec,
-                                                                   float(tf_rate) if teacher is not None else 1.0)
+                                                                   float(tf_rate) if teacher is not None else 1.0, ctc)
+                if ctc is not None and ctc.get('job') is not None:
+                    ctc_output._asr_ctc_job = ctc['job']
             if get_dec_state:
                 dec_state = hs[:, :, -1, :]
         if side_ctc and not ctc_async:
diff --git a/e2e-asr-pytorch_amd/src/functions.py b/e2e-asr-pytorch_amd/src/functions.py
--- a/e2e-asr-pytorch_amd/src/functions.py
+++ b/e2e-asr-pytorch_amd/src/functions.py
@@ -479,10 +479,49 @@
         return ga, None, gb, None
 
 
+def ctc_loss_buffers(logp, targets, input_len, target_len):
+    B, T, V = logp.shape
+    L = targets.shape[1]
+    dev = logp.device
+    nbytes = H.lib().asr_ctc_loss_workspace_bytes(B, T, L)
+    return {'logp': logp, 'L': L, 'nbytes': nbytes,
+            'nll': torch.empty(B, dtype=torch.float32, device=dev), 'loss': torch.empty((), dtype=torch.float32, device=dev),
+            'grad': _empty((B, T, V), logp), 'ws': torch.empty(nbytes, dtype=torch.uint8, device=dev),
+            'targets': targets.to(dev, torch.int64), 'il': input_len.to(dev, torch.int64).contiguous(),
+            'tl': target_len.to(dev, torch.int64).contiguous()}
+
+
+def attach_ctc_job(st, ctc):
+    logp, targets = ctc['logp'], ctc['targets']
+    if not (logp.is_cuda and logp.dim() == 3 and logp.is_contiguous() and logp.dtype == torch.float32 and targets.dim() == 2
+            and targets.is_contiguous() and 2 * targets.shape[1] + 1 <= 1024 and targets.shape[0] == logp.shape[0]):
+        return None
+    buf = ctc_loss_buffers(logp.detach(), targets, ctc['input_len'], ctc['target_len'])
+    st['ctc_job'] = H.ctc_job_struct(buf['logp'], buf['targets'], buf['il'], buf['tl'], buf['nll'], buf['loss'], buf['grad'], buf['L'],
+                                     1.0, buf['ws'])
+    buf['given'] = (targets, ctc['input_len'], ctc['target_len'])
+    return buf
+
+
+def _ctc_job_matches(job, logp, targets, input_len, target_len):
+    if not job or not job.get('ran'):
+        return False
+    def same(a, b):
+        return a is b or (torch.is_tensor(a) and torch.is_tensor(b) and a.device == b.device and a.data_ptr() == b.data_ptr()
+                          and a.shape == b.shape and a.dtype == b.dtype and a.stride() == b.stride())
+    g = job['given']
+    return (same(g[0], targets) and same(g[1], input_len) and same(g[2], target_len) and same(job['logp'], logp)
+            and logp._version == job['version'])
+
+
 class CTCLossFn(torch.autograd.Function):
     @staticmethod
-    def forward(ctx, logp_btv, targets, input_len, target_len):
+    def forward(ctx, logp_btv, targets, input_len, target_len, job=None):
         logp = logp_btv.contiguous()
+        if _ctc_job_matches(job, logp, targets, input_len, target_len):
+            ctx.save_for_backward(job['grad'])
+            ctx.nll = job['nll']
+            return job['loss']
         B, T, V = logp.shape
         targets = targets.contiguous()
         L = targets.shape[1]
@@ -507,7 +546,7 @@
     @staticmethod
     def backward(ctx, gout):
         (grad,) = ctx.saved_tensors
-        return scale_by_device_scalar(grad, gout), None, None, None
+        return scale_by_device_scalar(grad, gout), None, None, None, None
 
 
 class SeqLossFn(torch.autograd.Function):
@@ -643,7 +682,7 @@
     return ws
 
 
-def att_decoder_forward(model, enc, enc_len, L, teacher, prec):
+def att_decoder_forward(model, enc, enc_len, L, teacher, prec, ctc=None):
     B, Tp, _ = enc.shape
     d = _dec_dims(model, B, Tp, L)
     st = _dec_state(d, enc.device, half_copies=(prec == H.BF16 and d.E % 4 == 0))
@@ -652,6 +691,11 @@
         if nwork:
             st['work'] = _dec_workspace(model, 'fwd', (d.B, d.Tp, d.L), nwork, enc.device)
             H.abort_guard(st['work'])
+    job = None
+    if ctc is not None and st.get('work') is not None and ctc['logp'].dim() == 3 and ctc['targets'].dim() == 2:
+        _, T_ctc, V_ctc = ctc['logp'].shape
+        if int(H.lib().asr_att_decoder_fwd_ctc_roles(ctypes.byref(d), T_ctc, ctc['targets'].shape[1], V_ctc, None)) > 0:
+            job = attach_ctc_job(st, ctc)
     w = H.dec_weights_struct(_dec_tensors(model, False), d.NL)
     s = H.dec_state_struct(st)
     t_ptr, t_ld = (None, 0)
@@ -662,19 +706,23 @@
     H.call('asr_att_decoder_fwd', ctypes.byref(d), ctypes.byref(w), H.ptr(enc), H.ptr(enc_len), t_ptr, t_ld,
            ctypes.byref(s), prec, H.stream_ptr())
     H.watch_abort(st.get('work'))
+    if job is not None:
+        job['ran'] = bool(st.pop('ctc_job').ran)
+        job['version'] = ctc['logp']._version
+        ctc['job'] = job
     return d, st
 
 
 class AttDecoderFn(torch.autograd.Function):
     @staticmethod
-    def forward(ctx, anchor, enc, enc_len, teacher, L, model, prec, tf_rate=1.0):
+    def forward(ctx, anchor, enc, enc_len, teacher, L, model, prec, tf_rate=1.0, ctc=None):
         enc = enc.contiguous()
         enc_len = enc_len.to(enc.device, torch.int64).contiguous()
         if teacher is not None and tf_rate != 1:
             d, st = att_decoder_forward_sampled(model, enc, enc_len, L, teacher, prec, tf_rate, getattr(model, '_tf_decisions', None))
             model._last_tokens = st['tokens']
         else:
-            d, st = att_decoder_forward(model, enc, enc_len, L, teacher, prec)
+            d, st = att_decoder_forward(model, enc, enc_len, L, teacher, prec, ctc=ctc)
         ctx.model, ctx.prec, ctx.d, ctx.st = model, prec, d, st
         ctx.save_for_backward(enc, enc_len)
         att_seq = st['att'].view(d.B, 1, d.L, d.Tp)
@@ -719,7 +767,7 @@
                        ctypes.byref(s), H.ptr(dlogits), H.ptr(ws), nbytes, looped.value, prec, H.stream_ptr())
             H.defer_side(param_grads, enc, enc_len, dlogits, ws, *keep)
         ctx.st = None
-        return None, denc, None, None, None, None, None, None
+        return None, denc, None, None, None, None, None, None, None
 
 
 class EmbeddingFn(torch.autograd.Function):
diff --git a/e2e-asr-pytorch_amd/src/hipabi.py b/e2e-asr-pytorch_amd/src/hipabi.py
--- a/e2e-asr-pytorch_amd/src/hipabi.py
+++ b/e2e-asr-pytorch_amd/src/hipabi.py
@@ -27,9 +27,15 @@
                [(n, _vp * MAX_DEC_LAYERS) for n in ('Wih', 'Whh', 'bih', 'bhh')] + [('Wc', _vp), ('bc', _vp)]
 
 
+class CtcJob(ctypes.Structure):
+    _fields_ = ([(n, _vp) for n in ('logp', 'targets', 'input_len', 'target_len', 'nll', 'loss', 'grad')]
+                + [(n, ctypes.c_int) for n in ('B', 'T', 'V', 'L')]
+                + [('gscale', ctypes.c_float), ('workspace', _vp), ('workspace_bytes', ctypes.c_size_t), ('ran', ctypes.c_int)])
+
+
 class DecState(ctypes.Structure):
     _fields_ = ([(n, _vp) for n in ('key', 'att', 'q', 'xin', 'gates', 'cs', 'hs', 'logits', 'energy', 'conv', 'key16', 'enc16', 'work')]
-                + [('work_bytes', ctypes.c_size_t), ('tokens', _vp)])
+                + [('work_bytes', ctypes.c_size_t), ('tokens', _vp), ('ctc_job', ctypes.POINTER(CtcJob))])
 
 
 class BeamStep(ctypes.Structure):
@@ -212,6 +218,9 @@
     'asr_att_decoder_bwd_status_offset': (_sz, [_P(DecDims)]),
     'asr_att_decoder_bwd_persistent_tiles': (ctypes.c_int, [_P(DecDims)]),
     'asr_att_decoder_fwd_plan': (ctypes.c_int, [_P(DecDims)]),
+    'asr_att_decoder_fwd_ctc_roles': (ctypes.c_int, [_P(DecDims), _i, _i, _i, _P(_i)]),
+    'asr_att_decoder_set_ctc_roles': (ctypes.c_int, [_i]),
+    'asr_ctc_loss_launch_plan': (ctypes.c_int, [_i, _i, _i, _i, _P(ctypes.c_longlong)]),
     'asr_att_decoder_bwd_plan': (ctypes.c_int, [_P(DecDims)]),
     'asr_beam_attend_resident_max_t': (ctypes.c_int, [_i]),
 }
@@ -635,6 +644,16 @@
     return w
 
 
+def ctc_job_struct(logp, targets, input_len, target_len, nll, loss, grad, L, gscale, ws):
+    j = CtcJob()
+    j.logp, j.targets, j.input_len, j.target_len = logp.data_ptr(), targets.data_ptr(), input_len.data_ptr(), target_len.data_ptr()
+    j.nll, j.loss, j.grad = nll.data_ptr(), loss.data_ptr(), grad.data_ptr()
+    j.B, j.T, j.V = logp.shape
+    j.L, j.gscale = int(L), float(gscale)
+    j.workspace, j.workspace_bytes, j.ran = ws.data_ptr(), int(ws.numel()), 0
+    return j
+
+
 def dec_state_struct(tensors):
     s = DecState()
     for n, _ in DecState._fields_:
@@ -642,6 +661,10 @@
             w = tensors.get('work')
             s.work_bytes = int(w.numel() * w.element_size()) if w is not None else 0
             continue
+        if n == 'ctc_job':
+            j = tensors.get('ctc_job')
+            s.ctc_job = ctypes.pointer(j) if j is not None else None
+            continue
         t = tensors.get(n)
         setattr(s, n, t.data_ptr() if t is not None else None)
     return s
diff --git a/e2e-asr-pytorch_amd/src/step.py b/e2e-asr-pytorch_amd/src/step.py
--- a/e2e-asr-pytorch_amd/src/step.py
+++ b/e2e-asr-pytorch_amd/src/step.py
@@ -51,7 +51,8 @@
 def forward_losses(model, ctc_crit, att_crit, feat, feat_len, txt, decode_step, tf_rate, dp, txt_len, emb_decoder=None):
     from src import hipabi as H
     if emb_decoder is None:
-        ctc_output, encode_len, att_output, att_align, _ = model(feat, feat_len, decode_step, tf_rate=tf_rate, teacher=txt, ctc_async=True)
+        ctc_output, encode_len, att_output, att_align, _ = model(feat, feat_len, decode_step, tf_rate=tf_rate, teacher=txt, ctc_async=True,
+                                                                 ctc_target=(txt, txt_len))
         emb_loss = None
     else:
         if getattr(emb_decoder, 'apply_fuse', False) and tf_rate != 1:
@@ -71,7 +72,11 @@
                 ctc_loss = ctc_crit(ctc_output.transpose(0, 1), txt, encode_len, txt_len)
             H.join_branch(ctc_loss, ctc_output)
         else:
-            ctc_loss = ctc_crit(ctc_output.transpose(0, 1), txt, encode_len, txt_len)
+            lp_tbv = ctc_output.transpose(0, 1)
+            job = getattr(ctc_output, '_asr_ctc_job', None)
+            if job is not None:
+                lp_tbv._asr_ctc_job = job
+            ctc_loss = ctc_crit(lp_tbv, txt, encode_len, txt_len)
     w_att = None
     if att_output is not None:
         b, t, _ = att_output.shape
diff --git a/e2e-asr-pytorch_amd/src/util.py b/e2e-asr-pytorch_amd/src/util.py
--- a/e2e-asr-pytorch_amd/src/util.py
+++ b/e2e-asr-pytorch_amd/src/util.py
@@ -40,7 +40,8 @@
             input_lengths = torch.as_tensor(input_lengths)
         if not torch.is_tensor(target_lengths):
             target_lengths = torch.as_tensor(target_lengths)
-        return F_hip.CTCLossFn.apply(log_probs_tbv.transpose(0, 1), targets, input_lengths, target_lengths)
+        return F_hip.CTCLossFn.apply(log_probs_tbv.transpose(0, 1), targets, input_lengths, target_lengths,
+                                     getattr(log_probs_tbv, '_asr_ctc_job', None))
 
 
 class CrossEntropyLoss(nn.Module):
diff --git a/include/asr_hip.h b/include/asr_hip.h
--- a/include/asr_hip.h
+++ b/include/asr_hip.h
@@ -45,6 +45,7 @@
 int asr_lstm_bwd(float* gates, const float* whh, const float* dy, const float* c,
                  int B, int T, int H, int ND, int prec,
                  void* workspace, size_t workspace_bytes, asr_stream_t stream);
+int asr_ctc_loss_launch_plan(int B, int T, int V, int L, long long* out);
 
 size_t asr_lstm16_workspace_bytes(int B, int H, int ND, int backward);
 int asr_lstm16_fwd(void* gates16, const float* whh, void* y16, float* c, int B, int T, int H, int ND,
@@ -136,6 +137,15 @@
 } asr_dec_grads_t;
 
 typedef struct {
+    const float* logp; const int64_t* targets; const int64_t* input_len; const int64_t* target_len;
+    float *nll, *loss, *grad;
+    int B, T, V, L;
+    float gscale;
+    void* workspace; size_t workspace_bytes;
+    int ran;
+} asr_ctc_job_t;
+
+typedef struct {
     float* key;
     float* att;
     float* q;
@@ -151,6 +161,7 @@
     void* work;
     size_t work_bytes;
     int64_t* tokens;
+    asr_ctc_job_t* ctc_job;
 } asr_dec_state_t;
 
 int asr_att_decoder_fwd(const asr_dec_dims_t* dims, const asr_dec_weights_t* weights,
@@ -159,6 +170,8 @@
 size_t asr_att_decoder_bwd_workspace_bytes(const asr_dec_dims_t* dims);
 int asr_att_decoder_set_persistent(int flags);
 int asr_att_decoder_fwd_plan(const asr_dec_dims_t* dims);
+int asr_att_decoder_fwd_ctc_roles(const asr_dec_dims_t* dims, int T, int L_ctc, int V, int* plan);
+int asr_att_decoder_set_ctc_roles(int cap);
 int asr_att_decoder_bwd_plan(const asr_dec_dims_t* dims);
 int asr_att_decoder_energy_plan(const asr_dec_dims_t* dims, int* knmax, int* tpw);
 int asr_att_decoder_bwd_persistent_tiles(const asr_dec_dims_t* dims);
```

Result: no change. 1.155 million frames/s, median of 6 (+0.5%).
